# IvanTyulyandin/Spec_Viterbi

Measured on AMD Instinct MI355X. Metric: M state-updates/sec (states x obs/s) on 2405.chmm x emit_50_3500_20.ess, higher is better.
Workload: dtype f32; 1 GPU; 2405.chmm x emit_50_3500_20.ess, non-spec (min,+) step, diag kernel; states=2407, nnz=9621, sequences_per_gpu=50, observations_per_gpu=175000, state_updates_per_gpu=421225000, level=0, kernel=diag, threads=256, slots=1, fallback_rows=0, heavy_rows=2, golden_checked=False, checked_rows=0, parallelism=sequence-sharded x1 (one process per GPU, no collective)

## Files before the change

include/svh.h:

```cpp
#ifndef SPEC_VITERBI_SVH_H
#define SPEC_VITERBI_SVH_H

#include <stddef.h>
#include <stdint.h>

#ifdef __cplusplus
extern "C" {
#endif

#define SVH_ABI_VERSION 4

enum {
    SVH_OK = 0,
    SVH_E_INVALID = -1,
    SVH_E_RANGE = -2,
    SVH_E_NOMEM = -3,
    SVH_E_HIP = -4,
    SVH_E_UNSUPPORTED = -5,
    SVH_E_STATE = -6,
    SVH_E_IO = -7
};

typedef struct svh_hmm* svh_hmm_t;
typedef struct svh_ess* svh_ess_t;
typedef struct svh_model* svh_model_t;
typedef struct svh_batch* svh_batch_t;

int svh_abi_version(void);
const char* svh_last_error(void);
int svh_device_count(int* count);

int svh_hmm_read(const char* path, svh_hmm_t* out);
int svh_hmm_dims(svh_hmm_t h, uint64_t* n, uint64_t* S, uint64_t* nstart, uint64_t* ntrans);
int svh_hmm_copy(svh_hmm_t h, uint64_t* start_cols, float* start_vals, float* emissions,
                 uint64_t* trans_src, uint64_t* trans_dst, float* trans_prob);
void svh_hmm_free(svh_hmm_t h);
int svh_ess_read(const char* path, svh_ess_t* out);
int svh_ess_dims(svh_ess_t e, uint64_t* nseq, uint64_t* total_symbols);
int svh_ess_copy(svh_ess_t e, uint64_t* offsets , uint64_t* symbols);
void svh_ess_free(svh_ess_t e);

enum { SVH_KERNEL_AUTO = 0, SVH_KERNEL_FUSED = 1, SVH_KERNEL_GENERIC = 2, SVH_KERNEL_BAND = 3,
       SVH_KERNEL_CHAIN = 4, SVH_KERNEL_PIPE = 5, SVH_KERNEL_PIPE_WIDE = 6, SVH_KERNEL_SPEC2 = 7,
       SVH_KERNEL_SPEC2_PIPE = 8, SVH_KERNEL_DIAG = 9, SVH_KERNEL_SPEC2_DIAG = 10 };

typedef struct {
    int32_t device;
    int32_t kernel;
    int32_t max_threads;
    int32_t flags;
} svh_model_opts;

#define SVH_MODEL_SPEC_DENSE 1

int svh_model_create(uint64_t n, uint64_t S, uint64_t nstart, const uint64_t* start_cols,
                     const float* start_vals, const float* emissions, uint64_t ntrans,
                     const uint64_t* trans_src, const uint64_t* trans_dst,
                     const float* trans_prob, const svh_model_opts* opts, svh_model_t* out);
int svh_model_destroy(svh_model_t m);

typedef struct {
    int32_t kernel;
    int32_t family;
    int32_t threads;
    int32_t slots;
    int32_t light_terms;
    int32_t heavy_rows;
    int32_t heavy_uniform;
    int32_t device;
    uint64_t n, S, nnz;
    uint64_t lds_bytes;
    uint64_t spec_level;
    uint64_t spec_bytes;
    int32_t paths_kernel;
    int32_t wide_threads;
    int32_t wide_slots;
    uint32_t cu_count;
    int32_t pipe_slots;
    int32_t pipe_waves;
    int32_t pipe_groups;
    uint32_t pipe_max_nseq;
    int32_t pipew_slots;
    int32_t pipew_waves;
    int32_t pipew_blocks;
    uint32_t pipew_min_nseq;
    uint32_t pipe_max_nseq_paths;
    int32_t diag_ranges;
    uint32_t diag_max_nseq;
    int32_t diag_sm;
} svh_model_info;
int svh_model_get_info(svh_model_t m, svh_model_info* info);

int svh_spec_build(svh_model_t m, uint32_t level, void* stream);

enum { SVH_BATCH_PATHS = 1, SVH_BATCH_NO_TIMING = 2 };

int svh_batch_create(svh_model_t m, uint64_t nseq, const uint64_t* offsets,
                     const uint64_t* symbols, uint32_t flags, svh_batch_t* out);
int svh_batch_run(svh_batch_t b, uint32_t level, void* stream);
int svh_batch_run_time_parallel(svh_batch_t b, uint32_t seg_len, uint32_t probe_len, float rel_tol,
                                void* stream, uint64_t* fallbacks);
int svh_batch_read(svh_batch_t b, void* stream, float* scores ,
                   int64_t* best_state , int32_t* paths );
int svh_host_alloc(size_t bytes, void** out);
int svh_host_free(void* p);
int svh_batch_device_results(svh_batch_t b, float** scores, int64_t** best_state);
int svh_batch_elapsed_ms(svh_batch_t b, float* ms);
int svh_batch_step_floor_ms(svh_batch_t b, void* stream, uint32_t reps, float* ms);
int svh_batch_plan(svh_batch_t b, uint32_t level, svh_model_info* info);
int svh_batch_fallbacks(svh_batch_t b, uint64_t* rows);
int svh_batch_fallback_rows(svh_batch_t b, uint32_t* flags);
int svh_pipe_variant_built(int32_t slots, int32_t waves, int32_t table_mode, int32_t* built);
int svh_batch_destroy(svh_batch_t b);
int svh_batch_debug_fault(svh_batch_t b, void* stream);

int svh_batch_create_u8(svh_model_t m, uint64_t nseq, const uint64_t* offsets,
                        const uint8_t* symbols, uint32_t flags, svh_batch_t* out);

typedef struct svh_batchset* svh_batchset_t;
typedef struct {
    uint64_t members;
    uint64_t grouped;
    uint64_t launches;
    uint64_t grid;
    uint64_t lds_bytes;
    int32_t waves;
} svh_batchset_info;
int svh_batchset_create(const svh_model_t* models, uint64_t nmodels, uint64_t nseq,
                        const uint64_t* offsets, const uint8_t* symbols, uint32_t flags, svh_batchset_t* out);
int svh_batchset_run(svh_batchset_t s, uint32_t level, void* stream);
int svh_batchset_member(svh_batchset_t s, uint64_t i, svh_batch_t* out);
int svh_batchset_get_info(svh_batchset_t s, svh_batchset_info* info);
int svh_batchset_elapsed_ms(svh_batchset_t s, float* ms);
int svh_batchset_destroy(svh_batchset_t s);

enum { SVH_FORMAT_AUTO = 0, SVH_FORMAT_ESS = 1, SVH_FORMAT_FASTA = 2 };
typedef struct svh_reader* svh_reader_t;
int svh_reader_open(const char* path, int format, svh_reader_t* out);
int svh_reader_next(svh_reader_t r, uint64_t max_seqs, uint64_t max_symbols, uint64_t* nseq,
                    const uint64_t** offsets, const uint8_t** symbols);
void svh_reader_close(svh_reader_t r);

typedef int (*svh_result_fn)(void* user, uint64_t first_seq, uint64_t nseq, const uint64_t* offsets,
                             const float* scores, const int64_t* best_state, const int32_t* paths);
int svh_decode_file(svh_model_t m, const char* path, int format, uint32_t level, uint32_t flags,
                    uint64_t max_seqs, uint64_t max_symbols, svh_result_fn fn, void* user,
                    uint64_t* nseq_total);

int svh_viterbi(svh_model_t m, uint32_t level, uint64_t nseq, const uint64_t* offsets,
                const uint64_t* symbols, float* scores, int64_t* best_state, int32_t* paths);
int svh_viterbi_u8(svh_model_t m, uint32_t level, uint64_t nseq, const uint64_t* offsets,
                   const uint8_t* symbols, float* scores, int64_t* best_state, int32_t* paths);
int svh_viterbi_seqs(svh_model_t m, uint32_t level, uint64_t nseq, const uint64_t* const* seqs,
                     const uint64_t* lens, float* scores, int64_t* best_state, int32_t* paths);

#ifdef __cplusplus
}
#endif

#endif
```

spec_viterbi_amd/_lib.py:

```python
from __future__ import annotations

import ctypes
import os
from ctypes import POINTER, c_char_p, c_float, c_int, c_int32, c_int64, c_uint32, c_uint64, c_void_p

LIB_NAME = "libspec_viterbi_hip.so"
LIB_PATH = os.path.join(os.path.dirname(os.path.abspath(__file__)), LIB_NAME)
if os.environ.get("SVH_LIB"):
    LIB_PATH = os.path.abspath(os.environ["SVH_LIB"])

SVH_OK = 0
SVH_E_INVALID = -1
SVH_E_RANGE = -2
SVH_E_NOMEM = -3
SVH_E_HIP = -4
SVH_E_UNSUPPORTED = -5
SVH_E_STATE = -6
SVH_E_IO = -7

SVH_KERNEL_AUTO = 0
SVH_KERNEL_FUSED = 1
SVH_KERNEL_GENERIC = 2
SVH_KERNEL_BAND = 3
SVH_KERNEL_CHAIN = 4
SVH_KERNEL_PIPE = 5
SVH_KERNEL_PIPE_WIDE = 6
SVH_KERNEL_SPEC2 = 7
SVH_KERNEL_SPEC2_PIPE = 8
SVH_KERNEL_DIAG = 9
SVH_KERNEL_SPEC2_DIAG = 10
SVH_BATCH_PATHS = 1
SVH_BATCH_NO_TIMING = 2
SVH_MODEL_SPEC_DENSE = 1


class SvhError(RuntimeError):

    def __init__(self, code: int, msg: str):
        super().__init__(f"svh error {code}: {msg}")
        self.code = code


class svh_model_opts(ctypes.Structure):
    _fields_ = [("device", c_int32), ("kernel", c_int32), ("max_threads", c_int32), ("flags", c_int32)]


class svh_model_info(ctypes.Structure):
    _fields_ = [
        ("kernel", c_int32), ("family", c_int32), ("threads", c_int32), ("slots", c_int32),
        ("light_terms", c_int32), ("heavy_rows", c_int32), ("heavy_uniform", c_int32), ("device", c_int32),
        ("n", c_uint64), ("S", c_uint64), ("nnz", c_uint64), ("lds_bytes", c_uint64),
        ("spec_level", c_uint64), ("spec_bytes", c_uint64), ("paths_kernel", c_int32), ("wide_threads", c_int32),
        ("wide_slots", c_int32), ("cu_count", c_uint32), ("pipe_slots", c_int32), ("pipe_waves", c_int32),
        ("pipe_groups", c_int32), ("pipe_max_nseq", c_uint32),
        ("pipew_slots", c_int32), ("pipew_waves", c_int32), ("pipew_blocks", c_int32), ("pipew_min_nseq", c_uint32),
        ("pipe_max_nseq_paths", c_uint32),
        ("diag_ranges", c_int32),
        ("diag_max_nseq", c_uint32),
        ("diag_sm", c_int32),
    ]


class svh_batchset_info(ctypes.Structure):
    _fields_ = [("members", c_uint64), ("grouped", c_uint64), ("launches", c_uint64), ("grid", c_uint64),
                ("lds_bytes", c_uint64), ("waves", c_int32)]


P_u64 = POINTER(c_uint64)
P_f32 = POINTER(c_float)
P_i64 = POINTER(c_int64)
P_i32 = POINTER(c_int32)
P_u32 = POINTER(c_uint32)

SIGNATURES = {
    "svh_abi_version": (c_int, []),
    "svh_last_error": (c_char_p, []),
    "svh_device_count": (c_int, [P_i32]),
    "svh_hmm_read": (c_int, [c_char_p, POINTER(c_void_p)]),
    "svh_hmm_dims": (c_int, [c_void_p, P_u64, P_u64, P_u64, P_u64]),
    "svh_hmm_copy": (c_int, [c_void_p, P_u64, P_f32, P_f32, P_u64, P_u64, P_f32]),
    "svh_hmm_free": (None, [c_void_p]),
    "svh_ess_read": (c_int, [c_char_p, POINTER(c_void_p)]),
    "svh_ess_dims": (c_int, [c_void_p, P_u64, P_u64]),
    "svh_ess_copy": (c_int, [c_void_p, P_u64, P_u64]),
    "svh_ess_free": (None, [c_void_p]),
    "svh_model_create": (c_int, [c_uint64, c_uint64, c_uint64, P_u64, P_f32, P_f32, c_uint64, P_u64,
                                 P_u64, P_f32, POINTER(svh_model_opts), POINTER(c_void_p)]),
    "svh_model_destroy": (c_int, [c_void_p]),
    "svh_model_get_info": (c_int, [c_void_p, POINTER(svh_model_info)]),
    "svh_spec_build": (c_int, [c_void_p, c_uint32, c_void_p]),
    "svh_batch_create": (c_int, [c_void_p, c_uint64, P_u64, P_u64, c_uint32, POINTER(c_void_p)]),
    "svh_batch_run": (c_int, [c_void_p, c_uint32, c_void_p]),
    "svh_batch_read": (c_int, [c_void_p, c_void_p, P_f32, P_i64, P_i32]),
    "svh_host_alloc": (c_int, [ctypes.c_size_t, POINTER(c_void_p)]),
    "svh_host_free": (c_int, [c_void_p]),
    "svh_batch_device_results": (c_int, [c_void_p, POINTER(c_void_p), POINTER(c_void_p)]),
    "svh_batch_elapsed_ms": (c_int, [c_void_p, P_f32]),
    "svh_batch_step_floor_ms": (c_int, [c_void_p, c_void_p, c_uint32, P_f32]),
    "svh_batch_fallback_rows": (c_int, [c_void_p, P_u32]),
    "svh_batch_plan": (c_int, [c_void_p, c_uint32, POINTER(svh_model_info)]),
    "svh_batch_fallbacks": (c_int, [c_void_p, P_u64]),
    "svh_pipe_variant_built": (c_int, [ctypes.c_int32, ctypes.c_int32, ctypes.c_int32, POINTER(ctypes.c_int32)]),
    "svh_batch_debug_fault": (c_int, [c_void_p, c_void_p]),
    "svh_batch_destroy": (c_int, [c_void_p]),
    "svh_viterbi": (c_int, [c_void_p, c_uint32, c_uint64, P_u64, P_u64, P_f32, P_i64, P_i32]),
    "svh_viterbi_u8": (c_int, [c_void_p, c_uint32, c_uint64, P_u64, POINTER(ctypes.c_uint8), P_f32, P_i64, P_i32]),
    "svh_viterbi_seqs": (c_int, [c_void_p, c_uint32, c_uint64, P_u64, P_u64, P_f32, P_i64, P_i32]),
    "svh_batch_create_u8": (c_int, [c_void_p, c_uint64, P_u64, POINTER(ctypes.c_uint8), c_uint32, POINTER(c_void_p)]),
    "svh_batch_run_time_parallel": (c_int, [c_void_p, c_uint32, c_uint32, c_float, c_void_p, P_u64]),
    "svh_batchset_create": (c_int, [POINTER(c_void_p), c_uint64, c_uint64, P_u64, POINTER(ctypes.c_uint8), c_uint32,
                                    POINTER(c_void_p)]),
    "svh_batchset_run": (c_int, [c_void_p, c_uint32, c_void_p]),
    "svh_batchset_member": (c_int, [c_void_p, c_uint64, POINTER(c_void_p)]),
    "svh_batchset_get_info": (c_int, [c_void_p, POINTER(svh_batchset_info)]),
    "svh_batchset_elapsed_ms": (c_int, [c_void_p, P_f32]),
    "svh_batchset_destroy": (c_int, [c_void_p]),
    "svh_reader_open": (c_int, [c_char_p, c_int, POINTER(c_void_p)]),
    "svh_reader_next": (c_int, [c_void_p, c_uint64, c_uint64, P_u64, POINTER(P_u64),
                                POINTER(POINTER(ctypes.c_uint8))]),
    "svh_reader_close": (None, [c_void_p]),
    "svh_decode_file": (c_int, [c_void_p, c_char_p, c_int, c_uint32, c_uint32, c_uint64, c_uint64, c_void_p,
                                c_void_p, P_u64]),
}

SVH_FORMAT_AUTO, SVH_FORMAT_ESS, SVH_FORMAT_FASTA = 0, 1, 2
RESULT_FN = ctypes.CFUNCTYPE(c_int, c_void_p, c_uint64, c_uint64, P_u64, P_f32, P_i64, P_i32)


def _load():
    if not os.path.exists(LIB_PATH):
        raise ImportError(
            f"{LIB_PATH} not found: build the HIP extension first (python -c 'import __graft_entry__ as g; g.build()' "
            "or `make -j16`). There is no CPU fallback.")
    try:
        import torch
    except ImportError:
        pass
    lib = ctypes.CDLL(LIB_PATH)
    for name, (res, args) in SIGNATURES.items():
        fn = getattr(lib, name)
        fn.restype = res
        fn.argtypes = args
    return lib


lib = _load()


def check(rc: int) -> None:
    if rc != SVH_OK:
        msg = lib.svh_last_error()
        raise SvhError(rc, msg.decode() if msg else "")


def device_count() -> int:
    c = c_int32(0)
    check(lib.svh_device_count(ctypes.byref(c)))
    return int(c.value)


def pipe_variant_built(slots: int, waves: int, table_mode: int) -> bool:
    r = ctypes.c_int32()
    check(lib.svh_pipe_variant_built(slots, waves, table_mode, ctypes.byref(r)))
    return bool(r.value)
```

spec_viterbi_amd/csrc/diag.hip:

```cpp
#include "pipe_kernel.h"

#include <algorithm>
#include <cstdlib>

namespace svh {

namespace {

#ifndef SVH_DIAG_K
#define SVH_DIAG_K 64
#endif
constexpr uint32_t kDK = SVH_DIAG_K;
static_assert(kDK == 32 || kDK == 64, "block length");
constexpr uint32_t kDR = 5 * kDK;
constexpr uint32_t kDRS = kDR + 64;
constexpr uint32_t kDRS2 = kDR + 128;
static_assert(kDRS2 % 64 == 0, "the eb plane and the second diagonal lie whole multiples of 64 floats behind the lane's ea");
constexpr uint32_t kDG = kDR / kDK;
constexpr uint32_t kCP = kDK / 2;
constexpr uint32_t kDE = 4;
constexpr uint32_t kAG = 4;
#ifndef SVH_DIAG_PS
#define SVH_DIAG_PS 6
#endif
#ifndef SVH_DIAG_PE
#define SVH_DIAG_PE 2
#endif
constexpr uint32_t kPS = SVH_DIAG_PS;
constexpr uint32_t kPE = SVH_DIAG_PE;
constexpr uint32_t kNS = kPS + 2;
constexpr uint32_t kNE = kPE + 2;
static_assert(kPE + 2 <= kPS && kPS % 2 == 0 && kPE % 2 == 0 && kDK % kNS == 0 && kDK % kNE == 0,
              "prefetch distances: the register slots of step j (j % kNS, j % kNE) repeat every block");
static_assert(kPE == 2 && kDK % (2 * kAG) == 0,
              "address groups: read 2 kAG steps ahead into two register slots (group % 2), which repeat every block; "
              "a group's slot is free once the pairs of its last two steps are issued (kPE = 2)");
constexpr uint32_t kDMaxSym = 32;
static_assert(kDMaxSym == kDiagSetMaxSym, "kernels.h: what the runtime admits to a set launch");
#ifndef SVH_DIAG_AB
#define SVH_DIAG_AB 0
#endif
#ifndef SVH_DIAG_FINISH
#define SVH_DIAG_FINISH 0
#endif
#ifndef SVH_DIAG_PAB
#define SVH_DIAG_PAB 0
#endif
#ifndef SVH_DIAG_CMPX2
#define SVH_DIAG_CMPX2 1
#endif
#ifndef SVH_DIAG_LDPRIO
#define SVH_DIAG_LDPRIO 0
#endif
#ifndef SVH_DIAG_LDDRAIN
#define SVH_DIAG_LDDRAIN 1
#endif
#ifndef SVH_DIAG_DONE_STRIDE
#define SVH_DIAG_DONE_STRIDE 1
#endif

__device__ __forceinline__ f2 lds_ld2(uint32_t a) {
    return *(const __attribute__((address_space(3))) f2*)(size_t)a;
}
__device__ __forceinline__ float lds_ld1(uint32_t a) {
    return *(const __attribute__((address_space(3))) float*)(size_t)a;
}

__device__ __forceinline__ void check_off(float a, float b) {
    asm volatile("v_cmpx_nlt_f32_e32 vcc, %0, %1" : : "v"(a), "v"(b) : "vcc");
}
__device__ __forceinline__ void exec_collect(uint64_t& alive) {
    __builtin_amdgcn_sched_barrier(0);
    asm volatile("s_and_b64 %0, %0, exec\n\t"
                 "s_mov_b64 exec, -1\n\t"
                 "s_nop 4"
                 : "+s"(alive)
                 :
                 : "scc", "memory");
    __builtin_amdgcn_sched_barrier(0);
}

__host__ __device__ constexpr size_t diag_lds_main(uint32_t W, uint32_t S, bool sx, uint32_t dm = 1, bool ld = false) {
    return ((size_t)S * (dm == 2 ? kDRS2 : kDRS) * 2 + (size_t)S * 8 + (size_t)W * (ld ? 3 : 2) * kDK * (kDE + 1 + (sx ? 1 : 0)) + 2 * W) * 4;
}

constexpr uint32_t kFS = 8;
static_assert(kDK % kFS == 0 && 32 % kFS == 0 && kFS * 8 == 64, "fold: lane l reduces 8 lanes of step l / 8");
__host__ __device__ constexpr size_t diag_lds_paths(uint32_t W, uint32_t S, bool sx) {
    return ((diag_lds_main(W, S, sx) + 15) & ~(size_t)15) + (size_t)W * kFS * 64 * 4;
}

template <int W, bool SX, bool PATHS = false, int DM = 1, bool LD = false, bool FL = false>
__global__ __launch_bounds__(64 * (W + (LD ? 1 : 0))) __attribute__((amdgpu_waves_per_eu(2)))
void diag_viterbi_kernel(PipeModel m, FusedBatch b, PipeScratch x) {
    const uint32_t bx = blockIdx.x;
#include "diag_body.h"
}

template <class T>
__device__ __forceinline__ void in_global1(T*& p) {
    auto g = (__attribute__((address_space(1))) T*)p;
    asm volatile("" : "+s"(g));
    p = (T*)g;
}
template <class... T>
__device__ __forceinline__ void in_global(T*&... p) {
    (in_global1(p), ...);
}
template <int W>
__global__ __launch_bounds__(64 * W) __attribute__((amdgpu_waves_per_eu(2)))
void diag_set_kernel(const DiagSetEntry* __restrict__ e, const uint32_t* __restrict__ first, uint32_t ne) {
    constexpr bool SX = false, PATHS = false, LD = false, FL = false;
    constexpr int DM = 1;
    const uint32_t lane = threadIdx.x & 63u, gbx = blockIdx.x;
    uint32_t cnt = 0;
    for (uint32_t i0 = 0; i0 < ne; i0 += 64) {
        const uint32_t i = i0 + lane;
        const bool le = i < ne && first[i] <= gbx;
        const uint32_t c = (uint32_t)__builtin_popcountll(__builtin_amdgcn_ballot_w64(le));
        cnt += c;
        if (c < 64) break;
    }
    if (cnt == 0) return;
    const uint32_t i = (uint32_t)uniform((int)(cnt - 1));
    const uint32_t f0 = first[i];
    DiagSetEntry ent = e[i];
    in_global(ent.m.tab, ent.m.e0, ent.m.start, ent.m.lrow, ent.m.hc, ent.m.dtab, ent.m.pflags, ent.m.spos, ent.m.stamps, ent.m.dtab2);
    in_global(ent.b.symbols, ent.b.sym_off, ent.b.begin, ent.b.end, ent.b.v_in, ent.b.v_in_row, ent.b.scores, ent.b.best,
              ent.b.run_mask, ent.b.fault);
    in_global(ent.x.ctr, ent.x.done, ent.x.part, ent.x.gran, ent.x.cons, ent.x.viol, ent.x.xcc);
    const PipeModel& m = ent.m;
    const FusedBatch& b = ent.b;
    const PipeScratch& x = ent.x;
    const uint32_t bx = gbx - f0;
    {
#include "diag_body.h"
    }
}

template <bool SX>
__global__ __launch_bounds__(256) void diag_finish_kernel(PipeModel m, FusedBatch b, PipeScratch x) {
    extern __shared__ __attribute__((aligned(16))) float lds[];
    const uint32_t q = blockIdx.x, tid = threadIdx.x, lane = tid & 63u;
    uint32_t* flag = reinterpret_cast<uint32_t*>(lds + 2 * (size_t)m.P + 8);
    if (tid < 64) {
        float C = kInf, bv = kInf;
        uint32_t bk = kNoRow, vi = 0;
        for (uint32_t u = lane; u < m.nrng; u += 64) {
            const uint64_t* pu = x.part + ((size_t)q * x.G + u) * 2;
            const uint64_t a = pu[0], k2 = pu[1];
            C = fminf(C, __builtin_bit_cast(float, (uint32_t)a));
            vi |= (uint32_t)(a >> 32);
            if (k2 != ~0ull) lex_min(bv, bk, lex_key_value(k2), lex_key_index(k2));
        }
        C = wave_min63(C);
        wave_lexmin63(bv, bk);
        const bool any = __builtin_amdgcn_ballot_w64(vi != 0) != 0;
        if (lane == 63) {
            float* out = b.scores + (size_t)q * m.n;
            if (m.rowF >= 0) lex_min(bv, bk, out[m.rowF], (uint32_t)m.rowF);
            if (m.rowS >= 0) {
                out[m.rowS] = C;
                lex_min(bv, bk, C, (uint32_t)m.rowS);
            }
            if (b.best) b.best[q] = bk == kNoRow ? -1 : (int64_t)bk;
            x.viol[q] = any ? 1u : 0u;
            *flag = any ? 1u : 0u;
        }
    }
    __syncthreads();
    if (*flag) pipe_rerun_row<2, 4, SX>(m, b, q, lds);
}

template <int W, int DM = 1>
const void* diag_ptr(bool sx) {
    return sx ? reinterpret_cast<const void*>(&diag_viterbi_kernel<W, true, false, DM>)
              : reinterpret_cast<const void*>(&diag_viterbi_kernel<W, false, false, DM>);
}
template <int W, int DM>
const void* diag_loader_ptr(bool sx) {
    if constexpr (SVH_DIAG_AB != 0 || SVH_DIAG_FINISH != 0) {
        return nullptr;
    } else {
        return sx ? reinterpret_cast<const void*>(&diag_viterbi_kernel<W, true, false, DM, true>)
                  : reinterpret_cast<const void*>(&diag_viterbi_kernel<W, false, false, DM, true>);
    }
}
template <int DM>
const void* diag_floor_ptr(bool sx) {
    if constexpr (SVH_DIAG_AB != 0 || SVH_DIAG_FINISH != 0) {
        return nullptr;
    } else {
        return sx ? reinterpret_cast<const void*>(&diag_viterbi_kernel<4, true, false, DM, true, true>)
                  : reinterpret_cast<const void*>(&diag_viterbi_kernel<4, false, false, DM, true, true>);
    }
}
template <int W>
const void* diag_paths_ptr() {
    static_assert(kDK == 64, "the path records' block layout (two mask words, two checkpoints per block)");
    return reinterpret_cast<const void*>(&diag_viterbi_kernel<W, false, true>);
}

}

uint32_t diag_waves_for(uint64_t nseq) { return nseq >= 4 ? 4u : nseq >= 2 ? 2u : 1u; }

static size_t diag_lds(uint32_t W, uint32_t S, uint32_t P, bool sx, uint32_t dm = 1, bool ld = false) {
    const size_t rerun = (2 * (size_t)P + 2 * W) * 4;
    const size_t mainb = diag_lds_main(W, S, sx, dm, ld);
    return mainb > rerun ? mainb : rerun;
}

size_t diag_lds_bytes(uint32_t W, uint32_t S, uint32_t P, uint32_t dm, bool ld) { return diag_lds(W, S, P, true, dm, ld); }

uint32_t diag_sm_for(const PipeModel& m, uint64_t nseq, bool resumed, bool paths) {
    if (paths || !m.dtab2 || !m.nrng2 || SVH_DIAG_AB != 0 || SVH_DIAG_FINISH != 0) return 1;
    if (m.dsm == 1 || m.dsm == 2) return m.dsm;
    if (resumed || !m.cus) return 1;
    const uint64_t W = diag_waves_for(nseq);
    return (nseq + W - 1) / W * W * m.nrng > 4ull * m.cus ? 2 : 1;
}

bool diag_loader_for(const PipeModel& m, uint64_t nseq, bool resumed, bool paths) {
    if (paths || !nseq || SVH_DIAG_AB != 0 || SVH_DIAG_FINISH != 0 || m.dld == 1) return false;
    const uint32_t W = diag_waves_for(nseq);
    const uint32_t dm = diag_sm_for(m, nseq, resumed, paths);
    if (diag_lds(W, m.S, m.P, m.sx != 0, dm, true) > 160 * 1024) return false;
    if (m.dld == 3) return W == 4;
    if (m.dld == 2) return true;
    return m.cus && (nseq + W - 1) / W * (dm == 2 ? m.nrng2 : m.nrng) <= m.cus;
}

size_t diag_paths_lds_bytes(uint32_t W, uint32_t S, bool sx) { return diag_lds_paths(W, S, sx); }

bool diag_paths_fit(uint32_t S, bool sx) {
    return !sx && SVH_DIAG_AB == 0 && SVH_DIAG_FINISH == 0 && kDK == 64 && S > 0 && S <= kDMaxSym &&
           diag_lds_paths(4, S, sx) <= kDiagPathsLdsMax;
}

hipError_t launch_diag(const PipeModel& m, const FusedBatch& b, const PipeScratch& x, hipStream_t stream) {
    const bool paths = b.cmask != nullptr;
    if (!m.dtab || m.nrng == 0 || m.SM != 2 || m.S == 0 || m.S > kDMaxSym || (size_t)m.nrng * 64 > m.P || m.wide ||
        b.run_mask || (b.v_in && !b.v_in_row) || !x.part || !x.done || !x.viol || b.nseq > x.rows || x.G < m.nrng)
        return hipErrorInvalidValue;
    if (paths && (!b.cmask_off || !b.ckpt || !b.ckpt_off || !b.fck || !b.fck_off || !b.hrec || !b.hrec_off || !b.prec ||
                  !b.prec_off || b.v_in || !m.ties_heavy || !diag_paths_fit(m.S, m.sx != 0)))
        return hipErrorInvalidValue;
    if (b.nseq == 0) return hipSuccess;
    const uint32_t W = diag_waves_for(b.nseq);
    const uint32_t dm = diag_sm_for(m, b.nseq, b.v_in != nullptr, paths);
    if (dm == 2 && ((size_t)m.nrng2 * 128 != m.P || x.G < m.nrng2)) return hipErrorInvalidValue;
    const bool sx = m.sx != 0;
    const bool ld = diag_loader_for(m, b.nseq, b.v_in != nullptr, paths);
    const void* fn = paths     ? (W == 4 ? diag_paths_ptr<4>() : W == 2 ? diag_paths_ptr<2>() : diag_paths_ptr<1>())
                     : ld && m.dld == 3 ? (dm == 2 ? diag_floor_ptr<2>(sx) : diag_floor_ptr<1>(sx))
                     : ld      ? (dm == 2 ? (W == 4 ? diag_loader_ptr<4, 2>(sx) : W == 2 ? diag_loader_ptr<2, 2>(sx) : diag_loader_ptr<1, 2>(sx))
                                          : (W == 4 ? diag_loader_ptr<4, 1>(sx) : W == 2 ? diag_loader_ptr<2, 1>(sx) : diag_loader_ptr<1, 1>(sx)))
                     : dm == 2 ? (W == 4 ? diag_ptr<4, 2>(sx) : W == 2 ? diag_ptr<2, 2>(sx) : diag_ptr<1, 2>(sx))
                               : (W == 4 ? diag_ptr<4>(sx) : W == 2 ? diag_ptr<2>(sx) : diag_ptr<1>(sx));
    size_t lds = paths ? diag_lds_paths(W, m.S, sx) : diag_lds(W, m.S, m.P, sx, dm, ld);
    if (lds > 160 * 1024) return hipErrorInvalidValue;
    const uint64_t grid = ((uint64_t)b.nseq + W - 1) / W * (dm == 2 ? m.nrng2 : m.nrng);
    if (grid > 0x7FFFFFFFull) return hipErrorInvalidValue;
    if (m.cus) {
        const uint64_t per_cu = (grid + m.cus - 1) / m.cus;
        if (per_cu * lds <= 160 * 1024) {
            const size_t cap = (160 * 1024 / per_cu) & ~(size_t)511;
            lds = cap > lds ? cap : lds;
        }
    }
    if (lds > 64 * 1024) {
        const hipError_t e = hipFuncSetAttribute(fn, hipFuncAttributeMaxDynamicSharedMemorySize, (int)lds);
        if (e != hipSuccess) return e;
    }
    PipeModel mm = m;
    FusedBatch bb = b;
    PipeScratch xx = x;
    void* args[] = {&mm, &bb, &xx};
    const hipError_t e = hipLaunchKernel(fn, dim3((uint32_t)grid), dim3(64 * (W + (ld ? 1 : 0))), args, lds, stream);
#if SVH_DIAG_FINISH
    if (e != hipSuccess) return e;
    const void* fin = m.sx ? reinterpret_cast<const void*>(&diag_finish_kernel<true>)
                           : reinterpret_cast<const void*>(&diag_finish_kernel<false>);
    return hipLaunchKernel(fin, dim3(b.nseq), dim3(256), args, (2 * (size_t)m.P + 8 + 1) * 4, stream);
#else
    return e;
#endif
}

hipError_t diag_set_plan(const DiagSetEntry* host, const uint32_t* first_host, uint32_t ne, DiagSetLaunch* out) {
    if (!host || !first_host || !out || ne == 0 || first_host[0] != 0 || SVH_DIAG_AB != 0 || SVH_DIAG_FINISH != 0)
        return hipErrorInvalidValue;
    const uint32_t nseq = host[0].b.nseq;
    if (nseq == 0) return hipErrorInvalidValue;
    const uint32_t W = diag_waves_for(nseq);
    size_t lds = 0;
    for (uint32_t i = 0; i < ne; ++i) {
        const PipeModel& m = host[i].m;
        const FusedBatch& b = host[i].b;
        const PipeScratch& x = host[i].x;
        if (!m.dtab || m.nrng == 0 || m.SM != 2 || m.S == 0 || m.S > kDMaxSym || (size_t)m.nrng * 64 > m.P || m.wide ||
            m.sx || b.run_mask || b.cmask || (b.v_in && !b.v_in_row) || !x.part || !x.done || !x.viol || b.nseq != nseq ||
            b.nseq > x.rows || x.G < m.nrng || !b.symbols || !b.sym_off || !b.begin || !b.end || !b.scores)
            return hipErrorInvalidValue;
        const uint64_t blocks = ((uint64_t)nseq + W - 1) / W * m.nrng;
        if (first_host[i + 1] < first_host[i] || (uint64_t)first_host[i + 1] - first_host[i] != blocks) return hipErrorInvalidValue;
        lds = std::max(lds, diag_lds(W, m.S, m.P, false));
    }
    if (first_host[ne] > 0x7FFFFFFFu || lds > 160 * 1024) return hipErrorInvalidValue;
    out->grid = first_host[ne];
    out->lds_bytes = lds;
    out->waves = W;
    return hipSuccess;
}

hipError_t launch_diag_set(const DiagSetEntry* host, const uint32_t* first_host, uint32_t ne, const DiagSetEntry* entries,
                           const uint32_t* first, uint32_t cus, hipStream_t stream) {
    DiagSetLaunch L{};
    const hipError_t pe = diag_set_plan(host, first_host, ne, &L);
    if (pe != hipSuccess) return pe;
    if (!entries || !first) return hipErrorInvalidValue;
    const void* fn = L.waves == 4   ? reinterpret_cast<const void*>(&diag_set_kernel<4>)
                     : L.waves == 2 ? reinterpret_cast<const void*>(&diag_set_kernel<2>)
                                    : reinterpret_cast<const void*>(&diag_set_kernel<1>);
    size_t lds = L.lds_bytes;
    if (cus) {
        const uint64_t per_cu = (L.grid + cus - 1) / cus;
        if (per_cu * lds <= 160 * 1024) {
            const size_t cap = (160 * 1024 / per_cu) & ~(size_t)511;
            lds = cap > lds ? cap : lds;
        }
    }
    if (lds > 64 * 1024) {
        const hipError_t e = hipFuncSetAttribute(fn, hipFuncAttributeMaxDynamicSharedMemorySize, (int)lds);
        if (e != hipSuccess) return e;
    }
    const DiagSetEntry* ea = entries;
    const uint32_t* fa = first;
    uint32_t na = ne;
    void* args[] = {&ea, &fa, &na};
    return hipLaunchKernel(fn, dim3((uint32_t)L.grid), dim3(64 * L.waves), args, lds, stream);
}

}
```

spec_viterbi_amd/csrc/diag_body.h:

```cpp
    static_assert(DM == 1 || (DM == 2 && !PATHS), "decoded paths keep one diagonal per lane");
    static_assert(!LD || (!PATHS && SVH_DIAG_AB == 0 && SVH_DIAG_FINISH == 0), "the loader wave: scores only");
    static_assert(!FL || LD, "the floor is a loader-wave launch");
    constexpr uint32_t NB = LD ? 3 : 2;
    extern __shared__ __attribute__((aligned(16))) float lds[];
    constexpr uint32_t RW = 64 * DM;
    constexpr uint32_t RS = DM == 2 ? kDRS2 : kDRS;
    const uint32_t S = m.S, NR = DM == 2 ? m.nrng2 : m.nrng, NP = NR * RW, P = m.P;
    float* ring = lds;
    float* hcr = ring + (size_t)S * RS * 2;
    float* strm = hcr + S * 8;
    float* adr = strm + W * NB * kDK * kDE;
    float* xsf = adr + W * NB * kDK;
    uint32_t* wnb = reinterpret_cast<uint32_t*>(xsf + (SX ? W * NB * kDK : 0));
    uint32_t* rrow = wnb + W;

    const uint32_t tid = threadIdx.x, lane = tid & 63u;
    const uint32_t w = (uint32_t)uniform((int)(tid >> 6));
    const uint32_t rg = bx % NR, grp = bx / NR;
    const uint32_t q = grp * W + w;
    const bool ldr = LD && w == W;
    constexpr bool flr = FL;
    const bool real = (!LD || w < W) && q < b.nseq;
    const uint32_t ring_a = lds_addr(ring);

    for (uint32_t i = tid; i < S * 8; i += 64 * (W + (LD ? 1 : 0))) {
        const uint32_t o = i >> 3, k = i & 7u;
        const float* h = m.hc + o * 8;
        float v = 0.0f;
        if (k == 0) v = h[1];
        else if (k == 1) v = h[0];
        else if (k == 2) v = h[3];
        else if (k == 3) v = h[2];
        else if (k == 4) v = SX ? h[4] : kInf;
        else if (k == 5) v = __builtin_bit_cast(float, ring_a + o * RS * 8u);
        hcr[i] = v;
    }

    const uint8_t* __restrict__ sym = b.symbols + (real ? b.sym_off[q] : 0);
    const uint32_t len = real ? (uint32_t)uniform((int)b.end[q]) : 0u;
    const uint32_t beg = real ? (uint32_t)uniform((int)b.begin[q]) : 0u;
    const uint32_t first = beg ? beg : 1u;
    const uint32_t nst = len > first ? len - first : 0u;
    const uint32_t nb = (nst + kDK - 1) / kDK;
    if (lane == 0 && (!LD || w < W)) {
        wnb[w] = nb;
        rrow[w] = kNoRow;
    }

    constexpr uint32_t kT = 64 * W;
    constexpr uint32_t kRep = (kCP * kDMaxSym + kT - 1) / kT;
    const uint32_t nchunk = kCP * S;
    typedef float lvec __attribute__((ext_vector_type(4 * kRep)));
    lvec lreg;
    auto gload = [&](uint32_t g) {
        const uint32_t c0 = (rg * RW + g * kDK) % NP;
#pragma unroll
        for (uint32_t r = 0; r < kRep; ++r) {
            const uint32_t k = min(tid + r * kT, nchunk - 1);
            const float4 v = DM == 2 ? *reinterpret_cast<const float4*>(m.dtab2 + (size_t)(k / (kCP / 2)) * NP + c0 + 4 * (k % (kCP / 2)))
                                     : *reinterpret_cast<const float4*>(m.dtab + (size_t)(k / kCP) * NP + c0 + 2 * (k % kCP));
            lreg[4 * r] = v.x;
            lreg[4 * r + 1] = v.y;
            lreg[4 * r + 2] = v.z;
            lreg[4 * r + 3] = v.w;
        }
    };
    auto lwrite = [&](uint32_t g) {
        const uint32_t s0 = (g % kDG) * kDK;
#pragma unroll
        for (uint32_t r = 0; r < kRep; ++r) {
            const uint32_t k = tid + r * kT;
            if (k < nchunk) {
                float* d = DM == 2 ? ring + (size_t)(k / (kCP / 2)) * kDRS2 + s0 + 4 * (k % (kCP / 2))
                                   : ring + ((size_t)(k / kCP) * kDRS + s0 + 2 * (k % kCP)) * 2;
                const float4 v = make_float4(lreg[4 * r], lreg[4 * r + 1], lreg[4 * r + 2], lreg[4 * r + 3]);
                *reinterpret_cast<float4*>(d) = v;
                if (s0 < RW) *reinterpret_cast<float4*>(d + kDR * (DM == 2 ? 1 : 2)) = v;
            }
        }
    };
    uint32_t symv = 0;
    auto symload = [&](uint32_t kb) {
        const uint32_t t = first + kb * kDK + lane;
        const uint32_t tc = t < len ? t : (len ? len - 1 : 0u);
        symv = (real && lane < kDK) ? (uint32_t)sym[tc] : 0u;
    };
    auto sbuild = [&](uint32_t kb) {
        if (lane < kDK) {
            const uint32_t o = symv < S ? symv : 0u;
            const float4 h0 = *reinterpret_cast<const float4*>(hcr + o * 8);
            const float2 h1 = *reinterpret_cast<const float2*>(hcr + o * 8 + 4);
            const uint32_t i = kb * kDK + 1 + lane;
            const uint32_t e = (w * 2 + (kb & 1u)) * kDK + lane;
            *reinterpret_cast<float4*>(strm + e * kDE) = h0;
            adr[e] = __builtin_bit_cast(float, __builtin_bit_cast(uint32_t, h1.y) + (i % kDR) * (DM == 2 ? 4u : 8u));
            if (SX) xsf[e] = h1.x;
        }
    };
    constexpr uint32_t kRepL = kCP * kDMaxSym / 64;
    typedef float lvecl __attribute__((ext_vector_type(LD ? 4 * kRepL : 4)));
    lvecl lregl = 0.0f;
    const uint8_t* lsym[W] = {};
    uint32_t llen[W] = {}, lfirst[W] = {}, lsymv[W] = {};
    bool lreal[W] = {};
    auto gloadl = [&](uint32_t g) {
        if constexpr (LD) {
            const uint32_t c0 = (rg * RW + g * kDK) % NP;
#pragma unroll
            for (uint32_t r = 0; r < kRepL; ++r) {
                if (r * 64 < nchunk) {
                    const uint32_t k = min(lane + r * 64, nchunk - 1);
                    const float4 v = DM == 2 ? *reinterpret_cast<const float4*>(m.dtab2 + (size_t)(k / (kCP / 2)) * NP + c0 + 4 * (k % (kCP / 2)))
                                             : *reinterpret_cast<const float4*>(m.dtab + (size_t)(k / kCP) * NP + c0 + 2 * (k % kCP));
                    lregl[4 * r] = v.x;
                    lregl[4 * r + 1] = v.y;
                    lregl[4 * r + 2] = v.z;
                    lregl[4 * r + 3] = v.w;
                }
            }
        }
    };
    auto lwritel = [&](uint32_t g) {
        if constexpr (LD) {
            const uint32_t s0 = (g % kDG) * kDK;
#pragma unroll
            for (uint32_t r = 0; r < kRepL; ++r) {
                const uint32_t k = lane + r * 64;
                if (k < nchunk) {
                    float* d = DM == 2 ? ring + (size_t)(k / (kCP / 2)) * kDRS2 + s0 + 4 * (k % (kCP / 2))
                                       : ring + ((size_t)(k / kCP) * kDRS + s0 + 2 * (k % kCP)) * 2;
                    const float4 v = make_float4(lregl[4 * r], lregl[4 * r + 1], lregl[4 * r + 2], lregl[4 * r + 3]);
                    *reinterpret_cast<float4*>(d) = v;
                    if (s0 < RW) *reinterpret_cast<float4*>(d + kDR * (DM == 2 ? 1 : 2)) = v;
                }
            }
        }
    };
    auto symloadl = [&](uint32_t kb) {
#pragma unroll
        for (int u = 0; u < W; ++u) {
            const uint32_t t = lfirst[u] + kb * kDK + lane;
            const uint32_t tc = t < llen[u] ? t : (llen[u] ? llen[u] - 1 : 0u);
            lsymv[u] = (lreal[u] && lane < kDK) ? (uint32_t)lsym[u][tc] : 0u;
        }
    };
    auto sbuildl = [&](uint32_t kb) {
        if (lane < kDK) {
            const uint32_t i = kb * kDK + 1 + lane;
            const uint32_t ro = (i % kDR) * (DM == 2 ? 4u : 8u);
            const uint32_t e0 = (kb % NB) * kDK + lane;
#pragma unroll
            for (int u = 0; u < W; ++u) {
                const uint32_t o = lsymv[u] < S ? lsymv[u] : 0u;
                const float4 h0 = *reinterpret_cast<const float4*>(hcr + o * 8);
                const float2 h1 = *reinterpret_cast<const float2*>(hcr + o * 8 + 4);
                const uint32_t e = u * NB * kDK + e0;
                *reinterpret_cast<float4*>(strm + e * kDE) = h0;
                adr[e] = __builtin_bit_cast(float, __builtin_bit_cast(uint32_t, h1.y) + ro);
                if (SX) xsf[e] = h1.x;
            }
        }
    };
    if constexpr (LD) {
        if (ldr) {
#pragma unroll
            for (int u = 0; u < W; ++u) {
                const uint32_t qu = grp * W + u;
                lreal[u] = qu < b.nseq;
                lsym[u] = b.symbols + (lreal[u] ? b.sym_off[qu] : 0);
                llen[u] = lreal[u] ? (uint32_t)uniform((int)b.end[qu]) : 0u;
                const uint32_t bu = lreal[u] ? (uint32_t)uniform((int)b.begin[qu]) : 0u;
                lfirst[u] = bu ? bu : 1u;
            }
        }
    }

#if SVH_DIAG_AB == 6
    return;
#endif
    if constexpr (LD) {
        if (ldr) {
            gloadl(4);
            symloadl(0);
        } else {
            gload(0);
            lwrite(0);
            gload(1);
            lwrite(1);
            gload(2);
            lwrite(2);
            gload(3);
            lwrite(3);
        }
        __syncthreads();
        if (ldr) {
            sbuildl(0);
            symloadl(1);
            sbuildl(1);
            symloadl(2);
            if (flr) {
                sbuildl(2);
                lwritel(4);
            }
        }
    } else {
#if SVH_DIAG_AB != 4
    gload(0);
    lwrite(0);
    gload(1);
    lwrite(1);
    gload(2);
    lwrite(2);
    gload(3);
    lwrite(3);
    gload(4);
#endif
    symload(0);
    __syncthreads();
    sbuild(0);
    symload(1);
    }

    const uint32_t Lg = rg * 64 + lane;
    const uint32_t nck = len ? (len - 1) / kDiagCkptEvery + 1 : 0u;
    uint32_t* dmq = nullptr;
    float *ckq = nullptr, *fckq = nullptr, *cckq = nullptr, *pmq = nullptr, *fr_wr = nullptr;
    const float* fr_rd = nullptr;
    uint32_t pcur = Lg;
    if constexpr (PATHS) {
        float* fring = lds + ((diag_lds_main(W, S, SX) + 15) & ~(size_t)15) / 4 + w * kFS * 64;
        fr_wr = fring + lane;
        fr_rd = fring + lane * 8;
        if (real) {
            dmq = b.cmask + b.cmask_off[q] + Lg;
            ckq = b.ckpt + b.ckpt_off[q];
            fckq = b.fck + b.fck_off[q];
            cckq = reinterpret_cast<float*>(b.hrec + b.hrec_off[q]) + (size_t)rg * nck;
            pmq = reinterpret_cast<float*>(b.prec) + b.prec_off[q] + (size_t)rg * len + (lane >> 3);
        }
    }

    float xv = kInf, xv2 = kInf, F = kInf, c = kInf;
    uint64_t alive = ~0ull;
    if (real && beg == 0) {
        const uint32_t o0 = (uint32_t)uniform((int)sym[0]);
        const uint32_t p = rg * RW + lane;
        xv = m.e0[(size_t)o0 * P + p] + m.start[p];
        if (DM == 2) xv2 = m.e0[(size_t)o0 * P + p + 64] + m.start[p + 64];
        F = m.rowF >= 0 ? m.hc[o0 * 8 + 5] + m.startF : kInf;
        c = (rg == 0 && lane == 0 && m.rowS >= 0) ? m.hc[o0 * 8 + 6] + m.startS : kInf;
    } else if (real) {
        const float* vin = b.v_in + (size_t)b.v_in_row[q] * m.n;
        const uint32_t r = m.lrow[rg * RW + lane];
        xv = r != kNoRow ? vin[r] : kInf;
        if (DM == 2) {
            const uint32_t r2 = m.lrow[rg * RW + 64 + lane];
            xv2 = r2 != kNoRow ? vin[r2] : kInf;
        }
        F = m.rowF >= 0 ? vin[m.rowF] : kInf;
        c = (rg == 0 && lane == 0 && m.rowS >= 0) ? vin[m.rowS] : kInf;
    }
    if constexpr (PATHS) {
        if (real) {
            ckq[Lg] = xv;
            float mu0 = xv, c0 = c;
            wave_min63x2(mu0, c0);
            if (lane == 63) {
                pmq[-7] = mu0;
                cckq[0] = c0;
            }
            if (rg == 0 && lane == 0) fckq[0] = F;
        }
    }
    __syncthreads();
    uint32_t nbmax = 0;
#pragma unroll
    for (int u = 0; u < W; ++u) nbmax = wnb[u] > nbmax ? wnb[u] : nbmax;
    nbmax = (uint32_t)uniform((int)nbmax);

    typedef float hvec __attribute__((ext_vector_type(4 * kNS)));
    typedef float avec __attribute__((ext_vector_type(2 * kAG)));
    typedef float evec __attribute__((ext_vector_type(2 * DM * kNE)));
    hvec hq;
    avec aq, xq;
    evec eq;
    auto spos = [&](uint32_t kb, uint32_t j) {
        if constexpr (LD) return (w * NB + (j < kDK ? kb : kb + 1) % NB) * kDK + j % kDK;
        const uint32_t e0 = (w * 2 + (kb & 1u)) * kDK;
        return (j < kDK ? e0 : e0 ^ kDK) + j % kDK;
    };
    auto sread = [&](uint32_t kb, uint32_t j, uint32_t slot) {
        const float4 h = *reinterpret_cast<const float4*>(strm + spos(kb, j) * kDE);
        hq[4 * slot] = h.x;
        hq[4 * slot + 1] = h.y;
        hq[4 * slot + 2] = h.z;
        hq[4 * slot + 3] = h.w;
    };
    auto gread = [&](avec& q, const float* src, uint32_t kb, uint32_t j) {
        const float4 g = *reinterpret_cast<const float4*>(src + spos(kb, j));
        const uint32_t slot = (j / kAG) % 2;
        q[4 * slot] = g.x;
        q[4 * slot + 1] = g.y;
        q[4 * slot + 2] = g.z;
        q[4 * slot + 3] = g.w;
    };
    auto eread = [&](uint32_t j) {
        const float roff = aq[j % (2 * kAG)];
        if constexpr (DM == 2) {
            const uint32_t a = __builtin_bit_cast(uint32_t, roff) + lane * 4u;
            eq[4 * (j % kNE)] = lds_ld1(a);
            eq[4 * (j % kNE) + 1] = lds_ld1(a + 256u);
            eq[4 * (j % kNE) + 2] = lds_ld1(a + kDRS2 * 4u);
            eq[4 * (j % kNE) + 3] = lds_ld1(a + kDRS2 * 4u + 256u);
            return;
        }
        const f2 e = lds_ld2(__builtin_bit_cast(uint32_t, roff) + lane * 8u);
        eq[2 * (j % kNE)] = e.x;
        eq[2 * (j % kNE) + 1] = e.y;
    };
#pragma unroll
    for (uint32_t j = 0; j < kPS; ++j) sread(0, j, j);
    gread(aq, adr, 0, 0);
    gread(aq, adr, 0, kAG);
    if (SX) gread(xq, xsf, 0, 0);
#pragma unroll
    for (uint32_t j = 0; j < kPE; ++j) eread(j);

    f2 FC = (f2){F, c};
    f2 XP = (f2){xv, 0.0f};
    uint32_t dw = 0;
    auto step = [&](const float4& h, float xs, const f2& e, uint32_t slot = 0) {
        const f2 Y = XP.xx + (f2){h.x, h.y};
        const f2 Wv = FC + (f2){h.z, h.w};
        const float za = e.x + FC.x;
        const float zb = e.y + XP.x;
        float cn = fminf(Wv.y, Y.y);
        if (SX) cn = fminf(cn, xs + FC.x);
        check_off(Y.x, Wv.x);
        if constexpr (PATHS && SVH_DIAG_PAB != 1) push_le(dw, za, zb);
        XP.x = fminf(zb, za);
        FC = (f2){Wv.x, cn};
        if constexpr (PATHS && SVH_DIAG_PAB != 2) fr_wr[slot * 64] = XP.x;
    };
    f2 X2 = (f2){xv, xv2};
    uint32_t nviol = 0;
    auto step2 = [&](const float4& h, float xs, const f2& ea, const f2& eb) {
        XP.x = fminf(X2.x, X2.y);
        const f2 Y = XP.xx + (f2){h.x, h.y};
        const f2 Wv = FC + (f2){h.z, h.w};
        const f2 za = ea + FC.xx;
        const f2 zb = eb + X2;
        float cn = fminf(Wv.y, Y.y);
        if (SX) cn = fminf(cn, xs + FC.x);
        if (SVH_DIAG_CMPX2) check_off(Y.x, Wv.x);
        else nviol += Y.x < Wv.x ? 1u : 0u;
        X2 = (f2){fminf(zb.x, za.x), fminf(zb.y, za.y)};
        FC = (f2){Wv.x, cn};
    };
    float4 fa0 = make_float4(kInf, kInf, kInf, kInf), fa1 = fa0;
    auto fold_read = [&]() {
        if (SVH_DIAG_PAB == 2) return;
        __builtin_amdgcn_fence(__ATOMIC_SEQ_CST, "wavefront");
        fa0 = *reinterpret_cast<const float4*>(fr_rd);
        fa1 = *reinterpret_cast<const float4*>(fr_rd + 4);
        __builtin_amdgcn_fence(__ATOMIC_SEQ_CST, "wavefront");
    };
    auto fold_min = [&](uint32_t t0, uint32_t n) {
        if (SVH_DIAG_PAB == 2) return;
        uint32_t tv = t0;
        float4 a0 = fa0, a1 = fa1;
        asm volatile("" : "+v"(tv), "+v"(a0.x), "+v"(a0.y), "+v"(a0.z), "+v"(a0.w), "+v"(a1.x), "+v"(a1.y), "+v"(a1.z), "+v"(a1.w));
        float mn = fminf(fminf(fminf(a0.x, a0.y), fminf(a0.z, a0.w)), fminf(fminf(a1.x, a1.y), fminf(a1.z, a1.w)));
        const uint32_t inf = 0x7f800000u;
        mn = fminf(mn, __builtin_bit_cast(float, dpp_u<0xB1>(__builtin_bit_cast(uint32_t, mn), inf)));
        mn = fminf(mn, __builtin_bit_cast(float, dpp_u<0x4E>(__builtin_bit_cast(uint32_t, mn), inf)));
        mn = fminf(mn, __builtin_bit_cast(float, dpp_u<0x141>(__builtin_bit_cast(uint32_t, mn), inf)));
        if ((lane & 7u) == 0 && (lane >> 3) < n) pmq[tv] = mn;
    };
    auto fold = [&](uint32_t t0, uint32_t n) {
        fold_read();
        fold_min(t0, n);
    };
    uint32_t dw0 = 0;
    float xs0 = kInf, fs0 = kInf, cs0 = kInf;
    auto keep32 = [&]() {
        dw0 = dw;
        xs0 = XP.x;
        fs0 = FC.x;
        cs0 = FC.y;
    };
    auto block_records = [&](uint32_t kb, uint32_t rem) {
        if (SVH_DIAG_PAB == 3) {
            asm volatile("" : : "v"(dw0), "v"(dw), "v"(xs0), "v"(fs0), "v"(cs0));
            return;
        }
        uint32_t kv = kb, pc = pcur;
        float cn1 = cs0, cn2 = FC.y;
        asm volatile("" : "+v"(kv), "+v"(pc), "+v"(cn1), "+v"(cn2));
        const uint32_t w0 = rem > 32 ? dw0 : dw << (32u - rem);
        dmq[(size_t)(2 * kv) * NP] = w0;
        if (rem > 32) dmq[(size_t)(2 * kv + 1) * NP] = dw << (64u - rem);
        if (rem >= 32) {
            const bool two = rem == 64;
            uint32_t p1 = pc + 32;
            p1 = p1 >= NP ? p1 - NP : p1;
            uint32_t p2 = p1 + 32;
            p2 = p2 >= NP ? p2 - NP : p2;
            const float x1 = rem > 32 ? xs0 : XP.x, f1 = rem > 32 ? fs0 : FC.x;
            float c1 = rem > 32 ? cn1 : cn2, c2 = cn2;
            ckq[(size_t)(2 * kv + 1) * NP + p1] = x1;
            if (two) ckq[(size_t)(2 * kv + 2) * NP + p2] = XP.x;
            wave_min63x2(c1, c2);
            if (lane == 63) {
                cckq[2 * kv + 1] = c1;
                if (two) cckq[2 * kv + 2] = c2;
            }
            if (rg == 0 && lane == 0) {
                fckq[2 * kv + 1] = f1;
                if (two) fckq[2 * kv + 2] = FC.x;
            }
            pcur = p2;
        }
    };
    auto blockwork = [&](uint32_t kb) {
        lwrite(kb + 4);
        gload(kb + 5);
        sbuild(kb + 1);
        symload(kb + 2);
    };
    auto block = [&](uint32_t kb) {
        __builtin_amdgcn_sched_barrier(0);
#pragma unroll
        for (uint32_t j = 0; j < kDK; ++j) {
            const uint32_t a = (SVH_DIAG_AB == 1 || FL) ? 0u : j % kNS, b2 = FL ? 0u : j % kNE;
            const float4 h = make_float4(hq[4 * a], hq[4 * a + 1], hq[4 * a + 2], hq[4 * a + 3]);
            const float xs = SX ? xq[(SVH_DIAG_AB == 1 || FL) ? 0u : j % (2 * kAG)] : 0.0f;
            const f2 e = DM == 2 ? (f2){eq[4 * b2], eq[4 * b2 + 1]} : (f2){eq[2 * b2], eq[2 * b2 + 1]};
            if (j % 2 == 0) {
                if (SVH_DIAG_AB != 1 && !FL) {
                    sread(kb, j + kPS, (j + kPS) % kNS);
                    sread(kb, j + kPS + 1, (j + kPS + 1) % kNS);
                }
                if (SVH_DIAG_AB != 2 && !FL) {
                    eread(j + kPE);
                    eread(j + kPE + 1);
                }
                if (SVH_DIAG_AB != 1 && !FL && j % kAG == 0) {
                    gread(aq, adr, kb, j + 2 * kAG);
                    if (SX) gread(xq, xsf, kb, j + kAG);
                }
                if (SVH_DIAG_AB == 0 && !FL) {
                    __builtin_amdgcn_s_waitcnt(0xC07F | (((SX ? 6 : 5) + (PATHS ? 2 : 0) + (DM == 2 ? 2 : 0)) << 8));
                    __builtin_amdgcn_sched_barrier(0);
                }
            }
            if constexpr (DM == 2) step2(h, xs, e, (f2){eq[4 * b2 + 2], eq[4 * b2 + 3]});
            else step(h, xs, e, j % kFS);
            if (j % 2 == 1) __builtin_amdgcn_sched_barrier(0);
            if constexpr (PATHS) {
                if (j % kFS == kFS - 1 && (SVH_DIAG_PAB != 4 || j == kDK - 1)) {
                    exec_collect(alive);
                    if (SVH_DIAG_PAB == 4) {
                        fold(kb * kDK + 1 + j - (kFS - 1), kFS);
                    } else {
                        if (j >= kFS) fold_min(kb * kDK + 1 + j - (2 * kFS - 1), kFS);
                        fold_read();
                        if (j == kDK - 1) fold_min(kb * kDK + 1 + j - (kFS - 1), kFS);
                    }
                    if (j == 31) keep32();
                    if (j == kDK - 1) block_records(kb, kDK);
                    __builtin_amdgcn_sched_barrier(0);
                }
            }
        }
        if constexpr (!PATHS) exec_collect(alive);
    };
    auto tail = [&](uint32_t kb, uint32_t rem) {
        const uint32_t e0 = LD ? (w * NB + kb % NB) * kDK : (w * 2 + (kb & 1u)) * kDK;
        if constexpr (PATHS) {
            for (uint32_t g0 = 0; g0 < rem; g0 += kFS) {
                const uint32_t n = rem - g0 < kFS ? rem - g0 : kFS;
                __builtin_amdgcn_sched_barrier(0);
                for (uint32_t j = g0; j < g0 + n; ++j) {
                    const float4 h = *reinterpret_cast<const float4*>(strm + (e0 + j) * kDE);
                    const float roff = adr[e0 + j];
                    step(h, SX ? xsf[e0 + j] : 0.0f, lds_ld2(__builtin_bit_cast(uint32_t, roff) + lane * 8u), j - g0);
                }
                exec_collect(alive);
                fold(kb * kDK + 1 + g0, n);
                if (g0 + n == 32 && rem > 32) keep32();
            }
            block_records(kb, rem);
            return;
        }
        __builtin_amdgcn_sched_barrier(0);
        for (uint32_t j = 0; j < rem; ++j) {
            const float4 h = *reinterpret_cast<const float4*>(strm + (e0 + j) * kDE);
            const float roff = adr[e0 + j];
            if constexpr (DM == 2) {
                const uint32_t a = __builtin_bit_cast(uint32_t, roff) + lane * 4u;
                step2(h, SX ? xsf[e0 + j] : 0.0f, (f2){lds_ld1(a), lds_ld1(a + 256u)},
                      (f2){lds_ld1(a + kDRS2 * 4u), lds_ld1(a + kDRS2 * 4u + 256u)});
            } else {
                step(h, SX ? xsf[e0 + j] : 0.0f, lds_ld2(__builtin_bit_cast(uint32_t, roff) + lane * 8u));
            }
        }
        exec_collect(alive);
    };

    if constexpr (LD) {
        if (ldr) {
            for (uint32_t k = 0; k < nbmax; ++k) {
                if (!flr) {
                    sbuildl(k + 2);
                    symloadl(k + 3);
                    lwritel(k + 4);
                    gloadl(k + 5);
                }
                lds_barrier();
            }
            return;
        }
        if (SVH_DIAG_LDPRIO) __builtin_amdgcn_s_setprio(SVH_DIAG_LDPRIO);
    }
    for (uint32_t k = 0; k < nbmax; ++k) {
        const uint32_t rem = k < nb ? nst - k * kDK : 0u;
        const bool full = k < nb && rem >= kDK;
        if constexpr (!LD) blockwork(k);
        if (k < nb) {
#ifdef SVH_DIAG_SIMPLE
            tail(k, rem >= kDK ? kDK : rem);
#else
            if (full) block(k);
            else tail(k, rem);
#endif
        }
        if (LD && !SVH_DIAG_LDDRAIN) asm volatile("s_barrier" ::: "memory");
        else if (SVH_DIAG_AB != 3) lds_barrier();
    }

    if (DM == 2 && !SVH_DIAG_CMPX2) alive &= __builtin_amdgcn_ballot_w64(nviol == 0);
    F = FC.x;
    c = FC.y;
    xv = DM == 2 ? X2.x : XP.x;
    xv2 = X2.y;

#if SVH_DIAG_AB == 5
    if (real && m.lrow[(rg * 64 + lane + nst) % NP] != kNoRow)
        g_st_score(b.scores + (size_t)q * m.n + m.lrow[(rg * 64 + lane + nst) % NP], xv);
    return;
#endif
#if SVH_DIAG_FINISH
    if (real) {
        float* out = b.scores + (size_t)q * m.n;
        const uint32_t r = m.lrow[(rg * 64 + lane + nst) % NP];
        float bv = kInf;
        uint32_t bk = kNoRow;
        if (r != kNoRow) {
            out[r] = xv;
            bv = xv;
            bk = r;
        }
        wave_lexmin63(bv, bk);
        const float cmin = wave_min63(c);
        const bool any_viol = alive != ~0ull;
        if (lane == 63) {
            uint64_t* part = x.part + ((size_t)q * x.G + rg) * 2;
            part[0] = ((uint64_t)(any_viol ? 1u : 0u) << 32) | __builtin_bit_cast(uint32_t, cmin);
            part[1] = lex_key(bv, bk);
            if (rg == 0 && m.rowF >= 0) out[m.rowF] = F;
        }
    }
    return;
#endif
    uint32_t last = 0;
    if (real) {
        float* out = b.scores + (size_t)q * m.n;
        const uint32_t pe = (rg * RW + lane + nst) % NP;
        const uint32_t r = m.lrow[pe];
        float bv = kInf;
        uint32_t bk = kNoRow;
        if (r != kNoRow) {
            g_st_score(out + r, xv);
            bv = xv;
            bk = r;
        }
        if constexpr (DM == 2) {
            const uint32_t r2 = m.lrow[pe + 64 >= NP ? pe + 64 - NP : pe + 64];
            if (r2 != kNoRow) {
                g_st_score(out + r2, xv2);
                lex_min(bv, bk, xv2, r2);
            }
        }
        wave_lexmin63(bv, bk);
        const float cmin = wave_min63(c);
        const bool any_viol = alive != ~0ull;
        if (lane == 63 && !flr) {
            uint64_t* part = x.part + ((size_t)q * x.G + rg) * 2;
            g_st64(part, ((uint64_t)(any_viol ? 1u : 0u) << 32) | __builtin_bit_cast(uint32_t, cmin));
            g_st64(part + 1, lex_key(bv, bk));
#if SVH_DIAG_AB == 7
            last = rg == NR - 1 ? 1u : 0u;
#else
            asm volatile("s_waitcnt vmcnt(0)" ::: "memory");
            const uint32_t d = __hip_atomic_fetch_add(x.done + (size_t)q * SVH_DIAG_DONE_STRIDE, 1u, __ATOMIC_RELAXED, __HIP_MEMORY_SCOPE_AGENT);
            last = d == NR - 1 ? 1u : 0u;
#endif
#if SVH_DIAG_AB == 8
            last = 0;
#endif
        }
        last = readlane_u(last, 63);
    }
    if (last) {
        float C = kInf, bv2 = kInf;
        uint32_t bk2 = kNoRow, vi = 0;
        for (uint32_t u = lane; u < NR; u += 64) {
            const uint64_t* pu = x.part + ((size_t)q * x.G + u) * 2;
            const uint64_t a = g_ld64(pu), k2 = g_ld64(pu + 1);
            C = fminf(C, __builtin_bit_cast(float, (uint32_t)a));
            vi |= (uint32_t)(a >> 32);
            if (k2 != ~0ull) lex_min(bv2, bk2, lex_key_value(k2), lex_key_index(k2));
        }
        C = wave_min63(C);
        wave_lexmin63(bv2, bk2);
        const bool any = __builtin_amdgcn_ballot_w64(vi != 0) != 0;
        if (lane == 63) {
            float* out = b.scores + (size_t)q * m.n;
            if (m.rowF >= 0) {
                out[m.rowF] = F;
                lex_min(bv2, bk2, F, (uint32_t)m.rowF);
            }
            if (m.rowS >= 0) {
                out[m.rowS] = C;
                lex_min(bv2, bk2, C, (uint32_t)m.rowS);
            }
            if (b.best) b.best[q] = bk2 == kNoRow ? -1 : (int64_t)bk2;
            x.viol[q] = any ? 1u : 0u;
            __hip_atomic_store(x.done + (size_t)q * SVH_DIAG_DONE_STRIDE, 0u, __ATOMIC_RELAXED, __HIP_MEMORY_SCOPE_AGENT);
            if (any && !PATHS) rrow[w] = q;
        }
    }
    if constexpr (PATHS) return;
    __syncthreads();
    uint32_t rq[W];
#pragma unroll
    for (int u = 0; u < W; ++u) rq[u] = rrow[u];
#pragma unroll
    for (int u = 0; u < W; ++u) {
        if (rq[u] != kNoRow) {
            __syncthreads();
            pipe_rerun_row<2, W, SX>(m, b, rq[u], lds);
        }
    }
```

spec_viterbi_amd/csrc/kernels.h:

```cpp
#pragma once

#include <hip/hip_runtime.h>

#include <cstddef>
#include <cstdint>

namespace svh {

constexpr int kMaxHeavy = 4;
constexpr int kMaxExc = 4;
constexpr int kMaxWaves = 16;
constexpr uint32_t kNoPred = 0xFFFFu;
constexpr uint32_t kSymChunk = 4096;
constexpr uint32_t kSymPad = 64;
constexpr int kMaxFusedThreads = 512;

enum HeavyMode : int { kHeavyGeneral = 0, kHeavyUniform = 1 };

struct FusedModel {
    const float* emis;
    const float* start;
    const uint32_t* lcol;
    const float* lval;
    const float* hval;
    const uint8_t* hvalid;
    const float* hmask;
    int hrow[kMaxHeavy];
    float hw[kMaxHeavy];
    uint32_t xk[kMaxHeavy][kMaxExc];
    float xw[kMaxHeavy][kMaxExc];
    uint32_t H;
    uint32_t n;
    uint32_t S;
    uint32_t slots;
    uint32_t estride;
    uint32_t vstride;
    uint32_t B;
};

constexpr uint32_t kFaultPipe = 1u, kFaultPipeWide = 2u, kFaultChain = 4u;

struct FusedBatch {
    const uint8_t* symbols;
    const uint64_t* sym_off;
    const uint32_t* begin;
    const uint32_t* end;
    const float* v_in;
    const uint32_t* v_in_row;
    float* scores;
    int64_t* best;
    uint16_t* bp;
    const uint64_t* bp_off;
    uint32_t* cmask;
    const uint64_t* cmask_off;
    uint32_t* hrec;
    const uint64_t* hrec_off;
    float* ckpt;
    const uint64_t* ckpt_off;
    float2* prec;
    const uint64_t* prec_off;
    float* fck;
    const uint64_t* fck_off;
    const uint32_t* run_mask;
    const struct PipeScratch* pipe;
    uint32_t* fault;
    uint32_t nseq;
};

constexpr int kBandHeavy = 2;
constexpr int kMaxBandThreads = 1024;
constexpr int kDefaultBandThreads = 512;
constexpr int kBandTailA = 0;
constexpr int kBandTailX = kBandHeavy;
constexpr int kBandTailE = kBandHeavy + kBandHeavy * kBandHeavy;
constexpr int kBandTail = 8;
constexpr int band_tail_x(int h, int k) { return kBandTailX + (h == k ? h : kBandHeavy + h); }
static_assert(kBandHeavy == 2, "band_tail_x assumes two heavy rows");
static_assert(kBandTailE + kBandHeavy <= kBandTail, "band row tail");

struct BandModel {
    const float* erows;
    const float* erows_t;
    const float* start;
    const float* aw;
    const float* bw;
    const uint32_t* lrow;
    int hrow[kBandHeavy];
    int hvalid[kBandHeavy];
    float hstart[kBandHeavy];
    uint32_t n, S, B, SM, erow, H;
    uint32_t ge;
    uint32_t dbg;
    unsigned long long* stamps;
    const uint8_t* pflags;
    const int32_t* spos;
    uint32_t hx_exist;
    uint32_t hl_exist;
    uint32_t ties_heavy;
};
constexpr int kBandStamps = 8;

constexpr int kChainMaxSym = 32;
constexpr int kChainMaxThreads = 512;
constexpr uint32_t kChainSymChunk = 32768;
constexpr int kChainRing = 8;
inline size_t chain_lds_bytes() {
    return (size_t)kChainMaxSym * kBandTail * sizeof(float) + (size_t)kChainRing * 2 * kMaxWaves * 8 +
           3 * kChainRing * 4 + 2 * kMaxWaves * sizeof(float) + kChainSymChunk;
}
bool chain_supported(int sm, int waves, int ha, bool ge);
bool chain_paths_supported(int sm, int waves);
hipError_t launch_chain(const BandModel& m, int ha, const FusedBatch& b, hipStream_t stream);
hipError_t launch_chain_traceback(const BandModel& m, const FusedBatch& b, const uint64_t* path_off,
                                  int32_t* paths, hipStream_t stream);
inline uint64_t chain_mask_words(uint64_t len, uint32_t waves, uint32_t sm) {
    return len > 1 ? (len - 1 + 31) / 32 * (uint64_t)sm * 64 * waves : 0;
}
constexpr uint32_t kPathRing = 64;
constexpr uint32_t kRecWords = 4;
inline size_t chain_path_lds_bytes() { return (size_t)kPathRing * kRecWords * 4; }
inline uint64_t chain_hrec_words(uint64_t len) { return len > 1 ? (len - 1) * kRecWords : 0; }
constexpr uint32_t kCkptEvery = 16;
inline uint64_t chain_ckpt_floats(uint64_t len, uint32_t sm, uint32_t threads) {
    return len ? ((len - 1) / kCkptEvery + 1) * (uint64_t)sm * threads : 0;
}

constexpr int kPipeRing = 32;
constexpr int kPipeGroup = 8;
constexpr int kPipeGRing = 256;
constexpr int kPipeAhead = 4;
constexpr int kPipeWindow = 1024;
struct PipeModel {
    const float2* tab;
    const float* e0;
    const float* start;
    const uint32_t* lrow;
    const float* hc;
    int rowF, rowS;
    float startF, startS;
    uint32_t n, S, P, nblk, SM, W, G;
    uint32_t cus;
    uint32_t sx;
    uint32_t tm;
    uint32_t wide;
    float emax2;
    const float2* dtab;
    uint32_t nrng;
    uint32_t rerun;
    const uint8_t* pflags;
    const int32_t* spos;
    uint32_t hx_exist;
    uint32_t hl_exist;
    uint32_t ties_heavy;
    unsigned long long* stamps;
    uint32_t diag;
    uint32_t dld;
    const float* dtab2;
    uint32_t nrng2;
    uint32_t dsm;
};
constexpr int kPipeStamps = 15;
constexpr uint32_t kCtrClass = 4, kCtrLeft = 12, kCtrWords = 16;
struct PipeScratch {
    uint32_t* ctr;
    uint32_t* done;
    uint64_t* part;
    uint64_t* gran;
    uint32_t* cons;
    uint32_t* viol;
    uint32_t* xcc;
    uint32_t xmap;
    uint32_t rows, G;
};
constexpr uint32_t kPairSymbols = 20;
__host__ __device__ inline size_t pipe_lds_bytes(uint32_t W, uint32_t S) {
    return ((size_t)W * kPipeRing * 64 + 16 + (size_t)S * 8 + (size_t)W * 4 + 4) * 4;
}
__host__ __device__ inline bool pipe_rerun_fits(uint32_t P, uint32_t W) {
    return 2ull * P + 2ull * W <= (size_t)W * kPipeRing * 64;
}
bool pipe_supported(int sm, int waves, bool sx);
bool pipe_tm_supported(int tm);
hipError_t launch_pipe(const PipeModel& m, const FusedBatch& b, const PipeScratch& x, hipStream_t stream,
                       bool step_floor = false);
hipError_t launch_pipe_l2(const PipeModel& m, const FusedBatch& b, const PipeScratch& x, hipStream_t stream);
bool pipe_l2_supported(const PipeModel& m);
bool pipe_paths_supported(int sm, int waves);
hipError_t launch_pipe_traceback(const PipeModel& m, const FusedBatch& b, const uint64_t* path_off, int32_t* paths,
                                 const uint32_t* skip, hipStream_t stream);
constexpr uint32_t kPipeTbMaxP = 2560;
inline uint64_t pipe_mask_words(uint64_t len, uint32_t nblk, uint32_t sm) {
    return len > 1 ? (len - 1 + 31) / 32 * (uint64_t)nblk * sm * 64 : 0;
}
__host__ __device__ inline uint32_t pipe_prec_parts(bool wide) { (void)wide; return 1u; }
inline uint64_t pipe_prec_count(uint64_t len, uint32_t nblk, uint32_t parts) { return (uint64_t)nblk * parts * len; }
inline uint64_t pipe_ckpt_floats(uint64_t len, uint32_t P) { return len ? ((len - 1) / kCkptEvery + 1) * (uint64_t)P : 0; }
inline uint64_t pipe_fck_floats(uint64_t len) { return len ? (len - 1) / 32 + 1 : 0; }
constexpr uint32_t kPRingStride = 132;
constexpr uint32_t kPPlane = 260;
constexpr uint32_t kPQuadStride = 520;
inline size_t pipe_path_lds_bytes(uint32_t W) { return (size_t)W * 8 * kPQuadStride * 4; }
uint32_t diag_waves_for(uint64_t nseq);
size_t diag_lds_bytes(uint32_t W, uint32_t S, uint32_t P, uint32_t dm = 1, bool ld = false);
uint32_t diag_sm_for(const PipeModel& m, uint64_t nseq, bool resumed, bool paths);
bool diag_loader_for(const PipeModel& m, uint64_t nseq, bool resumed, bool paths);
hipError_t launch_diag(const PipeModel& m, const FusedBatch& b, const PipeScratch& x, hipStream_t stream);
constexpr uint32_t kDiagSetMaxSym = 32;
struct DiagSetEntry {
    PipeModel m;
    FusedBatch b;
    PipeScratch x;
};
struct DiagSetLaunch {
    uint64_t grid;
    size_t lds_bytes;
    uint32_t waves;
};
hipError_t diag_set_plan(const DiagSetEntry* host, const uint32_t* first_host, uint32_t ne, DiagSetLaunch* out);
hipError_t launch_diag_set(const DiagSetEntry* host, const uint32_t* first_host, uint32_t ne, const DiagSetEntry* entries,
                           const uint32_t* first, uint32_t cus, hipStream_t stream);
bool diag_l2_supported(const PipeModel& m);
size_t diag_l2_lds_bytes(uint32_t W, uint32_t S);
hipError_t launch_diag_l2(const PipeModel& m, const FusedBatch& b, const PipeScratch& x, hipStream_t stream);
constexpr uint32_t kDiagCkptEvery = 32;
constexpr size_t kDiagPathsLdsMax = 80 * 1024;
inline uint64_t diag_mask_words(uint64_t len, uint32_t nrng) { return len > 1 ? (len - 1 + 31) / 32 * (uint64_t)nrng * 64 : 0; }
inline uint64_t diag_ckpt_floats(uint64_t len, uint32_t nrng) {
    return len ? ((len - 1) / kDiagCkptEvery + 1) * (uint64_t)nrng * 64 : 0;
}
inline uint64_t diag_mu_floats(uint64_t len, uint32_t nrng) { return (uint64_t)nrng * len; }
inline uint64_t diag_cck_floats(uint64_t len, uint32_t nrng) { return len ? ((len - 1) / 32 + 1) * (uint64_t)nrng : 0; }
size_t diag_paths_lds_bytes(uint32_t W, uint32_t S, bool sx);
bool diag_paths_fit(uint32_t S, bool sx);
hipError_t launch_diag_traceback(const PipeModel& m, const FusedBatch& b, const uint64_t* path_off, int32_t* paths,
                                 const uint32_t* skip, hipStream_t stream);

__host__ __device__ inline uint32_t pipew_chunks(uint32_t SM, bool sx) { return SM / 2 + 1 + (sx ? 1 : 0); }
inline size_t pipew_lds_bytes(uint32_t SM, uint32_t W, uint32_t S, bool sx, bool paths = false) {
    return (size_t)S * pipew_chunks(SM, sx) * 64 * 16 + (size_t)W * 8 * 64 * 4 + 16 +
           (paths ? (size_t)W * 8 * kPRingStride * 4 : 0);
}
bool pipew_supported(int sm, int waves, bool sx);
uint32_t pipew_paths_waves_max(uint32_t sm, uint32_t S, bool sx);
bool pipew_paths_supported(int sm, uint32_t S, bool sx);
inline uint32_t pipew_waves_for(const PipeModel& m, uint64_t nseq) {
    const uint64_t need = (nseq * m.nblk + m.cus - 1) / (m.cus ? m.cus : 1);
    static const uint32_t ws[] = {1, 2, 4, 8, 12, 16};
    uint32_t w = m.W;
    for (uint32_t c : ws)
        if (c >= need) {
            w = c < m.W ? c : m.W;
            break;
        }
    return w;
}
hipError_t launch_pipew(const PipeModel& m, const FusedBatch& b, const PipeScratch& x, hipStream_t stream);

struct CsrModel {
    const float* emis;
    const float* start;
    const uint32_t* rowptr;
    const uint32_t* col;
    const float* val;
    const uint32_t* row_of;
    uint32_t n;
    uint32_t S;
    uint32_t nnz;
};

enum FusedFamily : int {
    kFamR2Uni = 0,
    kFamR2 = 1,
    kFamR4 = 2,
    kFamR8 = 3,
    kFamR16 = 4,
    kNumFamilies = 5
};
int family_rmax(int fam);
int family_hmax(int fam);
int family_xmax(int fam);
int family_mode(int fam);
constexpr int kSlotChoices[] = {1, 2, 3, 4, 5, 6, 8, 10, 12, 16};
constexpr int kNumSlotChoices = 10;

const void* fused_kernel_r2uni(int smax, bool paths);
const void* fused_kernel_r2(int smax, bool paths);
const void* fused_kernel_r4(int smax, bool paths);
const void* fused_kernel_r8(int smax, bool paths);
const void* fused_kernel_r16(int smax, bool paths);

inline size_t fused_lds_bytes_for(int sm, uint32_t B, uint32_t vstride) {
    const size_t ndma = (size_t)(sm + 3) / 4;
    return (3 * (size_t)vstride + 3 * ndma * B * 4) * sizeof(float) +
           3 * kMaxHeavy * sizeof(uint64_t) + 2 * kMaxWaves * sizeof(float) + kSymChunk + 64 + 16;
}
inline size_t fused_lds_bytes(const FusedModel& m) {
    return fused_lds_bytes_for((int)m.slots, m.B, m.vstride);
}
constexpr size_t kMaxLdsBytes = 160 * 1024;

hipError_t launch_fused(const FusedModel& m, const FusedBatch& b, int fam, bool paths,
                        hipStream_t stream);
constexpr int kBandSlotChoices[] = {1, 2, 3, 4, 5, 6, 8, 10, 12, 16};
constexpr int kNumBandSlotChoices = 10;
inline size_t band_lds_bytes(uint32_t erow) {
    return (3 * (size_t)erow + 4 * kMaxWaves + 2 * kMaxWaves) * sizeof(float) + kSymChunk + 64 + 16;
}
hipError_t launch_band(const BandModel& m, int ha, const FusedBatch& b, hipStream_t stream);
size_t generic_lds_bytes(uint32_t n);
hipError_t launch_generic(const CsrModel& m, const FusedBatch& b, int threads, bool paths,
                          hipStream_t stream);
hipError_t launch_traceback(const FusedBatch& b, const uint64_t* path_off, int32_t* paths,
                            uint32_t n, hipStream_t stream);

hipError_t launch_spec_fold(const CsrModel& m, float* mfold, hipStream_t stream);
hipError_t launch_spec_densify(const CsrModel& m, const float* mfold, float* h1, uint32_t pstride,
                               hipStream_t stream);
hipError_t launch_spec_extend(const CsrModel& m, const float* mfold, const float* h_prev,
                              uint64_t kprev, float* h_new, uint32_t pstride, hipStream_t stream);
struct SpecChunkBatch {
    const uint8_t* symbols;
    const uint64_t* sym_off;
    const uint32_t* nchunks;
    const float* v_src;
    float* v_dst;
    uint32_t nseq;
    uint32_t level;
    uint32_t chunk;
};
hipError_t launch_spec_chunk(const CsrModel& m, const float* products, const SpecChunkBatch& c,
                             uint32_t pstride, hipStream_t stream);
constexpr uint32_t kSpec2Threads = 1024;
constexpr uint32_t kSpec2LightMax = 4;
struct Spec2Model {
    const float* emis;
    const uint32_t* la;
    const uint32_t* lb;
    const float* lv;
    const uint32_t* thr;
    const uint32_t* tcp;
    const uint32_t* ha;
    const uint32_t* hb;
    const float* hv;
    const uint32_t* hrow;
    const float* amax;
    uint32_t n, S, H, NP;
    uint32_t R, KL, NHS;
    uint32_t nhs;
    uint32_t prune;
    unsigned long long* stamps;
};
constexpr int kSpec2Stamps = 8;
struct Spec2Batch {
    const uint8_t* symbols;
    const uint64_t* sym_off;
    const uint32_t* len;
    const uint32_t* nchunks;
    float* v;
// ... 61 lines not shown
```

spec_viterbi_amd/csrc/runtime.cpp:

```cpp
#include "runtime.h"

#include <algorithm>
#include <chrono>
#include <cmath>
#include <cstdio>
#include <cstdlib>
#include <cstring>
#include <functional>
#include <limits>
#include <map>
#include <memory>
#include <numeric>

namespace svh {

namespace {

constexpr float kInfH = std::numeric_limits<float>::infinity();

uint32_t round_up(uint32_t x, uint32_t m) { return (x + m - 1) / m * m; }

uint32_t float_bits(float f) {
    uint32_t u;
    std::memcpy(&u, &f, 4);
// ... 494 lines not shown
    if (ge) {
        const uint32_t smp = (SM + 3) / 4 * 4;
        bp.erows_t.assign((size_t)S * B * smp, kInfH);
        for (uint32_t o = 0; o < S; ++o)
            for (uint32_t p = 0; p < nL; ++p)
                bp.erows_t[((size_t)o * B + p / SM) * smp + p % SM] = hm.emis[(size_t)o * n + light[p]];
    }
    bp.erows.assign((size_t)S * erow, kInfH);
    for (uint32_t o = 0; o < S; ++o) {
        const float* E = hm.emis.data() + (size_t)o * n;
        float* row = bp.erows.data() + (size_t)o * erow;
        for (uint32_t p = 0; p < nL; ++p) row[slot_of(p)] = E[light[p]];
        float* tl = row + cap;
        for (int x = 0; x < kBandHeavy; ++x) {
            if (!bp.hvalid[x]) continue;
            const float eh = E[bp.hrow[x]];
            tl[kBandTailA + x] = eh + wh[x];
            for (const auto& [src, w] : exc[x]) tl[band_tail_x((int)x, (int)src)] = eh + w;
            tl[kBandTailE + x] = eh;
        }
    }
    return bp;
}

void DeviceBandPlan::upload(const BandPlan& p, uint32_t n, uint32_t S, hipStream_t s) {
    plan = p;
    if (!p.ok) return;
    d_erows.upload(p.erows.data(), p.erows.size() * 4, s);
    d_start.upload(p.start.data(), p.start.size() * 4, s);
    d_aw.upload(p.aw.data(), p.aw.size() * 4, s);
    d_bw.upload(p.bw.data(), p.bw.size() * 4, s);
    d_lrow.upload(p.lrow.data(), p.lrow.size() * 4, s);
    if (p.ge) d_erows_t.upload(p.erows_t.data(), p.erows_t.size() * 4, s);
    d_pflags.upload(p.pflags.data(), p.pflags.size(), s);
    d_spos.upload(p.spos.data(), p.spos.size() * 4, s);
    std::memset(&view, 0, sizeof(view));
    view.erows = d_erows.as<float>();
    view.start = d_start.as<float>();
    view.aw = d_aw.as<float>();
    view.bw = d_bw.as<float>();
    view.lrow = d_lrow.as<uint32_t>();
    view.erows_t = p.ge ? d_erows_t.as<float>() : nullptr;
    view.ge = p.ge ? 1u : 0u;
    view.pflags = d_pflags.as<uint8_t>();
    view.spos = d_spos.as<int32_t>();
    view.hx_exist = p.hx_exist;
    view.hl_exist = p.hl_exist;
    view.ties_heavy = p.ties_heavy ? 1u : 0u;
    for (int h = 0; h < kBandHeavy; ++h) {
        view.hrow[h] = p.hrow[h];
        view.hvalid[h] = p.hvalid[h];
        view.hstart[h] = p.hstart[h];
    }
    view.n = n;
    view.S = S;
    view.B = p.B;
    view.SM = p.SM;
    view.erow = p.erow;
    view.H = p.H;
    const char* dbg = std::getenv("SVH_BAND_DEBUG");
    view.dbg = dbg ? (uint32_t)std::atoi(dbg) : 0u;
    if (view.dbg & (4u | 128u)) {
        d_stamps.alloc((size_t)4096 * kMaxWaves * kBandStamps * 8);
        hip_check(hipMemsetAsync(d_stamps.ptr, 0, d_stamps.bytes, s), "stamps");
        view.stamps = d_stamps.as<unsigned long long>();
    }
}

PipePlan make_pipe_plan(const HostModel& hm, uint32_t sm, uint32_t waves, bool wide) {
    PipePlan pp;
    const uint32_t n = hm.n, S = hm.S;
    if (S > 32) return pp;
    const BandShape sh = analyze_band(hm);
    if (!sh.ok || sh.HA != 1) return pp;
    const uint32_t H = (uint32_t)sh.heavy.size();
    float xff = kInfH, xss = kInfH, xsf = kInfH;
    for (const auto& e : sh.exc[0]) {
        if (e.first != 0) return pp;
        xff = e.second;
    }
    bool sx = false;
    if (H == 2) {
        for (const auto& e : sh.exc[1]) {
            if (e.first == 1) xss = e.second;
            else { xsf = e.second; sx = true; }
        }
    }
    if (const char* e = std::getenv(wide ? "SVH_PIPEW_SM" : "SVH_PIPE_SM")) sm = (uint32_t)std::atoi(e);
    if (const char* e = std::getenv(wide ? "SVH_PIPEW_WAVES" : "SVH_PIPE_WAVES")) waves = (uint32_t)std::atoi(e);
    if (sm == 0) sm = wide ? 8 : 2;
    if (waves == 0) waves = wide ? 16 : 4;
    if (wide ? !pipew_supported((int)sm, (int)waves, sx) : !pipe_supported((int)sm, (int)waves, sx)) return pp;
    if (wide && pipew_lds_bytes(sm, waves, S, sx) > 160 * 1024) return pp;
    const uint32_t nL = (uint32_t)sh.light.size();
    const uint32_t bsz = 64 * sm;
    pp.wide = wide;
    pp.SM = sm;
    pp.W = waves;
    pp.nblk = (nL + bsz - 1) / bsz;
    pp.G = wide ? pp.nblk : (pp.nblk + waves - 1) / waves;
    pp.P = pp.nblk * bsz;
    pp.sx = sx;
    pp.rowF = (int)sh.heavy[0];
    pp.rowS = H == 2 ? (int)sh.heavy[1] : -1;
    pp.startF = hm.start[sh.heavy[0]];
    pp.startS = H == 2 ? hm.start[sh.heavy[1]] : kInfH;
    const uint32_t P = pp.P;
    const uint32_t nc = wide ? pipew_chunks(sm, sx) : 0;
    pp.tab.assign(wide ? (size_t)pp.nblk * S * nc * 64 * 4 : (size_t)pp.nblk * S * sm * 64 * 2, kInfH);
    pp.e0.assign((size_t)S * P, kInfH);
    pp.start.assign(P, kInfH);
    pp.lrow.assign(P, 0xFFFFFFFFu);
    for (uint32_t p = 0; p < nL; ++p) {
        const uint32_t j = sh.light[p], blk = p / bsz, lane = (p % bsz) / sm, s = p % sm;
        pp.start[p] = hm.start[j];
        pp.lrow[p] = j;
        for (uint32_t o = 0; o < S; ++o) {
            const float e = hm.emis[(size_t)o * n + j];
            pp.e0[(size_t)o * P + p] = e;
            const float eb = e + sh.bw[p];
            const float ea = e + sh.aw[0][p];
            if (wide) {
                const uint32_t ib = s == 0 ? sm - 1 : s - 1, ia = sm + s;
                float* base = pp.tab.data() + (((size_t)blk * S + o) * nc) * 64 * 4;
                base[((ib / 4) * 64 + lane) * 4 + ib % 4] = eb;
                base[((ia / 4) * 64 + lane) * 4 + ia % 4] = ea;
            } else {
                float* t = pp.tab.data() + ((((size_t)blk * S + o) * sm + s) * 64 + lane) * 2;
                t[0] = eb;
                t[1] = ea;
            }
        }
    }
    if (!wide && sm == 2) {
        pp.nrng = (nL + 63) / 64;
        const uint32_t NP = pp.nrng * 64;
        pp.dtab.assign((size_t)S * NP * 2, kInfH);
        for (uint32_t p = 0; p < nL; ++p)
            for (uint32_t o = 0; o < S; ++o) {
                const float e = hm.emis[(size_t)o * n + sh.light[p]];
                float* d = pp.dtab.data() + ((size_t)o * NP + p) * 2;
                d[0] = e + sh.aw[0][p];
                d[1] = e + sh.bw[p];
            }
        pp.nrng2 = (nL + 127) / 128;
        const uint32_t NP2 = pp.nrng2 * 128;
        pp.dtab2.assign((size_t)S * 2 * NP2, kInfH);
        for (uint32_t p = 0; p < nL; ++p)
            for (uint32_t o = 0; o < S; ++o) {
                const float* d = pp.dtab.data() + ((size_t)o * NP + p) * 2;
                pp.dtab2[((size_t)o * 2) * NP2 + p] = d[0];
                pp.dtab2[((size_t)o * 2 + 1) * NP2 + p] = d[1];
            }
        if (sh.bw[0] < kInfH) {
            pp.nrng = pp.nrng2 = 0;
            pp.dtab.clear();
            pp.dtab2.clear();
        }
    }
    pp.pflags.assign(P, 0);
    pp.spos.assign(n, 0);
    pp.ties_heavy = nL > 0;
    for (uint32_t p = 0; p < nL; ++p) {
        uint8_t f = sh.bex[p] ? 1 : 0;
        if (sh.aex[0][p]) f |= 2;
        if (p > 0 && sh.heavy[0] < sh.light[p - 1]) f |= 4;
        pp.pflags[p] = f;
        pp.ties_heavy = pp.ties_heavy && (f & 2) && (!(f & 1) || (f & 4));
        pp.spos[sh.light[p]] = (int32_t)p;
    }
    for (uint32_t x = 0; x < H; ++x) pp.spos[sh.heavy[x]] = -1 - (int32_t)x;
    pp.hx_exist = sh.hx_exist;
    pp.hl_exist = sh.hl_exist;
    pp.hc.assign((size_t)S * 8, kInfH);
    auto wide_consts = [&](uint32_t o, const float* c) {
        for (uint32_t blk = 0; blk < pp.nblk; ++blk)
            for (uint32_t lane = 0; lane < 64; ++lane) {
                float* base = pp.tab.data() + ((((size_t)blk * S + o) * nc + sm / 2) * 64 + lane) * 4;
                for (int k = 0; k < 4; ++k) base[k] = c[k];
                if (sx) {
                    float* b2 = base + 64 * 4;
                    b2[0] = c[4];
                    b2[1] = b2[2] = b2[3] = 0.0f;
                }
            }
    };
    for (uint32_t o = 0; o < S; ++o) {
        float* c = pp.hc.data() + (size_t)o * 8;
        const float eF = hm.emis[(size_t)o * n + sh.heavy[0]];
        const float eS = H == 2 ? hm.emis[(size_t)o * n + sh.heavy[1]] : kInfH;
        c[0] = eS + (H == 2 ? sh.wh[1] : kInfH);
        c[1] = eF + sh.wh[0];
        c[2] = eS + xss;
        c[3] = eF + xff;
        c[4] = eS + xsf;
        c[5] = eF;
        c[6] = eS;
        c[7] = 0.0f;
        if (wide) wide_consts(o, c);
    }
    bool nonneg = !wide;
    for (float v : hm.val) nonneg = nonneg && v >= 0.0f;
    for (float v : hm.emis) nonneg = nonneg && v >= 0.0f;
    for (float v : hm.start) nonneg = nonneg && v >= 0.0f;
    pp.emax2 = nonneg ? 0.0f : kInfH;
    if (nonneg)
        for (uint32_t p = 0; p < nL; ++p)
            for (uint32_t o = 0; o < S; ++o) {
                const float ea = hm.emis[(size_t)o * n + sh.light[p]] + sh.aw[0][p];
                if (ea < kInfH) pp.emax2 = std::max(pp.emax2, ea);
            }
    pp.ok = true;
    return pp;
}

void DevicePipePlan::upload(const PipePlan& p, uint32_t n, uint32_t S, hipStream_t s) {
    plan = p;
    if (!p.ok) return;
    d_tab.upload(p.tab.data(), p.tab.size() * 4, s);
    d_e0.upload(p.e0.data(), p.e0.size() * 4, s);
    d_start.upload(p.start.data(), p.start.size() * 4, s);
    d_lrow.upload(p.lrow.data(), p.lrow.size() * 4, s);
    d_hc.upload(p.hc.data(), p.hc.size() * 4, s);
    d_pflags.upload(p.pflags.data(), p.pflags.size(), s);
    d_spos.upload(p.spos.data(), p.spos.size() * 4, s);
    std::memset(&view, 0, sizeof(view));
    view.pflags = d_pflags.as<uint8_t>();
    view.spos = d_spos.as<int32_t>();
    view.hx_exist = p.hx_exist;
    view.hl_exist = p.hl_exist;
    view.ties_heavy = p.ties_heavy ? 1u : 0u;
    view.tab = d_tab.as<float2>();
    view.e0 = d_e0.as<float>();
    view.start = d_start.as<float>();
    view.lrow = d_lrow.as<uint32_t>();
    view.hc = d_hc.as<float>();
    view.rowF = p.rowF;
    view.rowS = p.rowS;
    view.startF = p.startF;
    view.startS = p.startS;
    view.n = n;
    view.S = S;
    view.P = p.P;
    view.nblk = p.nblk;
    view.SM = p.SM;
    view.W = p.W;
    view.G = p.G;
    view.sx = p.sx ? 1u : 0u;
    view.wide = p.wide ? 1u : 0u;
    view.rerun = !p.wide && pipe_rerun_fits(p.P, p.W) ? 1u : 0u;
    if (p.nrng && !p.dtab.empty() && diag_lds_bytes(diag_waves_for(4), S, p.P) <= 160 * 1024) {
        d_dtab.upload(p.dtab.data(), p.dtab.size() * 4, s);
        view.dtab = d_dtab.as<float2>();
        view.nrng = p.nrng;
        if (p.nrng2 && !p.dtab2.empty() && (size_t)p.nrng2 * 128 == p.P &&
            diag_lds_bytes(diag_waves_for(4), S, p.P, 2) <= 160 * 1024) {
            d_dtab2.upload(p.dtab2.data(), p.dtab2.size() * 4, s);
            view.dtab2 = d_dtab2.as<float>();
            view.nrng2 = p.nrng2;
        }
        if (const char* e = std::getenv("SVH_DIAG_SM")) {
            const int v = std::atoi(e);
            view.dsm = v == 1 || v == 2 ? (uint32_t)v : 0u;
        }
        if (const char* e = std::getenv("SVH_DIAG_LOADER"); e && *e) view.dld = std::atoi(e) ? 2u : 1u;
    }
    view.emax2 = p.emax2;
    view.tm = !p.wide && p.SM == 2 && (p.W == 4 || (p.W == 8 && pipe_tm_supported(-8))) && S <= kPairSymbols ? 4u : 0u;
    if (const char* e = std::getenv("SVH_PIPE_TM"); e) {
        const int t = std::atoi(e);
        if (t == 0 || (t >= 1 && t <= 4 && view.tm && pipe_tm_supported(t))) view.tm = (uint32_t)t;
    }
    if (const char* e = std::getenv("SVH_PIPE_DEBUG"); e && std::atoi(e)) {
        d_stamps.alloc((size_t)65536 * kPipeStamps * 8);
        hip_check(hipMemsetAsync(d_stamps.ptr, 0, d_stamps.bytes, s), "stamps");
        view.stamps = d_stamps.as<unsigned long long>();
        view.diag = (uint32_t)std::atoi(e) >> 1;
    }
}

void DevicePipePlan::report_stamps(uint32_t nseq) const {
    if (!view.stamps) return;
    const size_t waves = (size_t)nseq * plan.G * plan.W;
    if (waves > 65536 / kPipeStamps * kPipeStamps) return;
    std::vector<unsigned long long> h(waves * kPipeStamps);
    if (hipMemcpy(h.data(), view.stamps, h.size() * 8, hipMemcpyDeviceToHost) != hipSuccess) return;
    double sum[kPipeStamps] = {}, mx[kPipeStamps] = {};
    for (size_t w = 0; w < waves; ++w)
        for (int k = 0; k < kPipeStamps; ++k) {
            sum[k] += (double)h[w * kPipeStamps + k];
            mx[k] = std::max(mx[k], (double)h[w * kPipeStamps + k]);
        }
    std::fprintf(stderr, "pipe stamps (avg / max per wave): loop %.0f/%.0f head %.0f/%.0f tail %.0f/%.0f "
                 "prev %.0f/%.0f next %.0f/%.0f gran %.0f/%.0f cons %.0f/%.0f iters %.0f slow-groups %.0f/%.0f\n",
                 sum[0] / waves, mx[0], sum[1] / waves, mx[1], sum[2] / waves, mx[2], sum[3] / waves, mx[3],
                 sum[4] / waves, mx[4], sum[5] / waves, mx[5], sum[6] / waves, mx[6], sum[7] / waves,
                 sum[14] / waves, mx[14]);
    {
        unsigned long long t0 = ~0ull, tend = 0;
        for (size_t w = 0; w < waves; ++w)
            if (h[w * kPipeStamps + 8]) {
                t0 = std::min(t0, h[w * kPipeStamps + 8]);
                tend = std::max(tend, h[w * kPipeStamps + 11]);
            }
        if (t0 != ~0ull) std::fprintf(stderr, "pipe wall (us from first entry): last sweep end %.2f\n", (tend - t0) * 0.01);
        for (uint32_t q = 0; t0 != ~0ull && q < nseq; ++q) {
            std::fprintf(stderr, "  seq %u:", q);
            for (uint32_t g = 0; g < plan.G; ++g) {
                unsigned long long en = 0, st = 0, ed = 0, tb = 0;
                for (uint32_t w = 0; w < plan.W; ++w) {
                    const unsigned long long* r = h.data() + (((size_t)q * plan.G + g) * plan.W + w) * kPipeStamps;
                    if (!r[8]) continue;
                    en = std::max(en, r[8] - t0);
                    if (w == 0) st = r[9] - t0;
                    if (w == 0 && r[13]) tb = r[13] - t0;
                    ed = std::max(ed, r[11] - t0);
                }
                const unsigned long long* r0 = h.data() + (((size_t)q * plan.G + g) * plan.W) * kPipeStamps;
                const unsigned long long hw = r0[12];
                const double mhz = r0[10] > r0[9] ? (double)r0[0] / ((double)(r0[10] - r0[9]) * 0.01) : 0.0;
                std::fprintf(stderr, " [g%u in %.1f tab %.1f st %.1f end %.1f x%u s%u c%u %.0fMHz]", g, en * 0.01, tb * 0.01,
                             st * 0.01, ed * 0.01, (unsigned)(hw >> 32) & 0xFu, (unsigned)(hw >> 13) & 0x3u,
                             (unsigned)(hw >> 8) & 0xFu, mhz);
            }
            std::fprintf(stderr, "\n");
        }
        for (size_t w = 0; t0 != ~0ull && w < waves; ++w) {
            const unsigned long long* r = h.data() + w * kPipeStamps;
            if (!r[8] || w / plan.W >= 2 * plan.G) continue;
            std::fprintf(stderr, "  wave %zu (seq-ticket %zu): entry %.2f start %.2f body_end %.2f end %.2f\n", w % plan.W,
                         w / plan.W, (r[8] - t0) * 0.01, (r[9] - t0) * 0.01, (r[10] - t0) * 0.01, (r[11] - t0) * 0.01);
        }
    }
    {
        std::fprintf(stderr, "pipe wait split by role (mean over %u rows): g w loop prev next gran cons slow\n", nseq);
        for (uint32_t g = 0; g < plan.G; ++g)
            for (uint32_t w = 0; w < plan.W; ++w) {
                double a[8] = {};
                uint32_t cnt = 0;
                for (uint32_t q = 0; q < nseq; ++q) {
                    const unsigned long long* r = h.data() + (((size_t)q * plan.G + g) * plan.W + w) * kPipeStamps;
                    if (!r[8]) continue;
                    ++cnt;
                    a[0] += (double)r[0];
                    for (int k = 3; k <= 6; ++k) a[k - 2] += (double)r[k];
                    a[5] += (double)r[14];
                }
                if (!cnt) continue;
                std::fprintf(stderr, "  role g%u w%u: %.0f %.1f %.1f %.1f %.1f %.1f\n", g, w, a[0] / cnt, a[1] / cnt,
                             a[2] / cnt, a[3] / cnt, a[4] / cnt, a[5] / cnt);
            }
    }
    uint32_t qlast = 0;
    unsigned long long elast = 0;
    for (uint32_t q = 0; q < nseq; ++q)
        for (size_t w = 0; w < (size_t)plan.G * plan.W; ++w)
            if (h[((size_t)q * plan.G * plan.W + w) * kPipeStamps + 11] > elast) {
                elast = h[((size_t)q * plan.G * plan.W + w) * kPipeStamps + 11];
                qlast = q;
            }
    for (uint32_t q : {0u, qlast}) {
        for (uint32_t g = 0; g < plan.G; ++g)
            for (uint32_t w = 0; w < plan.W; ++w) {
                const unsigned long long* r = h.data() + (((size_t)q * plan.G + g) * plan.W + w) * kPipeStamps;
                std::fprintf(stderr, "  seq %u g%u w%u: loop %llu head %llu tail %llu prev %llu next %llu gran %llu cons %llu slow %llu\n",
                             q, g, w, r[0], r[1], r[2], r[3], r[4], r[5], r[6], r[14]);
            }
        if (qlast == 0) break;
    }
}

void PipeScratchBuffers::ensure(uint32_t rows, uint32_t G, hipStream_t s) {
    if (!d_ctr.ptr) {
        d_ctr.alloc(kCtrWords * 4);
        hip_check(hipMemsetAsync(d_ctr.ptr, 0, kCtrWords * 4, s), "pipe counters");
    }
    if (view.ctr && rows <= view.rows && G <= view.G) return;
    rows = std::max(rows, view.rows);
    G = std::max(G, view.G);
    auto zeroed = [&](DeviceBuffer& d, size_t bytes) {
        d.alloc(bytes);
        hip_check(hipMemsetAsync(d.ptr, 0, d.bytes, s), "pipe scratch");
    };
    zeroed(d_done, (size_t)rows * 128);
    zeroed(d_part, (size_t)rows * G * 16);
    zeroed(d_gran, (size_t)rows * std::max<uint32_t>(G - 1, 1) * kPipeGRing * 8);
    zeroed(d_cons, (size_t)rows * G * 8);
    zeroed(d_viol, (size_t)rows * 4);
    zeroed(d_xcc, (size_t)rows * G * 4);
    view.ctr = d_ctr.as<uint32_t>();
    view.done = d_done.as<uint32_t>();
    view.part = d_part.as<uint64_t>();
    view.gran = d_gran.as<uint64_t>();
    view.cons = d_cons.as<uint32_t>();
    view.viol = d_viol.as<uint32_t>();
    view.xcc = d_xcc.as<uint32_t>();
    view.rows = rows;
    view.G = G;
}

void PipeScratchBuffers::note_launch(hipStream_t s) {
    if (launches > 0 && launches % kEpochSpan == 0) {
        hip_check(hipMemsetAsync(d_ctr.ptr, 0, d_ctr.bytes, s), "pipe epoch reset");
        hip_check(hipMemsetAsync(d_gran.ptr, 0, d_gran.bytes, s), "pipe epoch reset");
        hip_check(hipMemsetAsync(d_cons.ptr, 0, d_cons.bytes, s), "pipe epoch reset");
        hip_check(hipMemsetAsync(d_xcc.ptr, 0, d_xcc.bytes, s), "pipe epoch reset");
    }
    ++launches;
}

void DeviceBandPlan::report_stamps(uint32_t nseq) const {
    if (!(view.dbg & (4u | 128u)) || !view.stamps) return;
    std::vector<unsigned long long> h((size_t)nseq * kMaxWaves * kBandStamps);
    if (hipMemcpy(h.data(), view.stamps, h.size() * 8, hipMemcpyDeviceToHost) != hipSuccess) return;
    double sum[kBandStamps] = {};
    uint32_t cnt = 0;
    for (uint32_t q = 0; q < nseq; ++q)
        for (uint32_t w = 0; w < std::max<uint32_t>(plan.B / 64, 1); ++w, ++cnt)
// ... 269 lines not shown
        for (uint32_t k = 0; k < nt; ++k) {
            sp.thr[t + k] = h;
            sp.tcp[t + k] = n * sp.KL + cpoff[h];
        }
        t += nt;
    }
    sp.amax.assign(H, 0.0f);
    bool nonneg = true;
    for (uint32_t j = 0; j < n; ++j)
        for (uint32_t e = hm.rowptr[j]; e < hm.rowptr[j + 1]; ++e) {
            nonneg = nonneg && hm.val[e] >= 0.0f;
            const int32_t h = hid[hm.col[e]];
            if (h < 0) continue;
            for (uint32_t o = 0; o < S; ++o) {
                const float a = hm.emis[(size_t)o * n + j] + hm.val[e];
                if (a < kInfH) sp.amax[h] = std::max(sp.amax[h], a);
            }
        }
    for (float e : hm.emis) nonneg = nonneg && e >= 0.0f;
    for (float e : hm.start) nonneg = nonneg && e >= 0.0f;
    sp.prune = nonneg;
    if (H == 0) {
        sp.hrow.push_back(0);
        sp.amax.push_back(0.0f);
    }
    sp.ok = true;
    return sp;
}

void DeviceSpec2Plan::upload(const Spec2Plan& p, const HostModel& hm, const float* d_emis, hipStream_t s) {
    plan = p;
    std::memset(&view, 0, sizeof(view));
    if (!p.ok) return;
    d_la.upload(p.la.data(), p.la.size() * 4, s);
    d_lb.upload(p.lb.data(), p.lb.size() * 4, s);
    d_lv.upload(p.lv.data(), p.lv.size() * 4, s);
    d_thr.upload(p.thr.data(), p.thr.size() * 4, s);
    d_tcp.upload(p.tcp.data(), p.tcp.size() * 4, s);
    d_ha.upload(p.ha.data(), p.ha.size() * 4, s);
    d_hb.upload(p.hb.data(), p.hb.size() * 4, s);
    d_hv.upload(p.hv.data(), p.hv.size() * 4, s);
    d_hrow.upload(p.hrow.data(), p.hrow.size() * 4, s);
    d_amax.upload(p.amax.data(), p.amax.size() * 4, s);
    view.emis = d_emis;
    view.la = d_la.as<uint32_t>();
    view.lb = d_lb.as<uint32_t>();
    view.lv = d_lv.as<float>();
    view.thr = d_thr.as<uint32_t>();
    view.tcp = d_tcp.as<uint32_t>();
    view.ha = d_ha.as<uint32_t>();
    view.hb = d_hb.as<uint32_t>();
    view.hv = d_hv.as<float>();
    view.hrow = d_hrow.as<uint32_t>();
    view.amax = d_amax.as<float>();
    view.n = hm.n;
    view.S = hm.S;
    view.H = p.H;
    view.NP = p.NP;
    view.R = p.R;
    view.KL = p.KL;
    view.NHS = p.NHS;
    view.nhs = p.nhs;
    view.prune = p.prune ? 1u : 0u;
    if (const char* e = std::getenv("SVH_SPEC2_DEBUG"); e && std::atoi(e)) {
        d_stamps.alloc((size_t)4096 * 16 * kSpec2Stamps * 8);
        hip_check(hipMemsetAsync(d_stamps.ptr, 0, d_stamps.bytes, s), "stamps");
        view.stamps = d_stamps.as<unsigned long long>();
    }
}

void DeviceSpec2Plan::report_stamps(uint32_t nseq) const {
    if (!view.stamps) return;
    nseq = std::min<uint32_t>(nseq, 4096);
    std::vector<unsigned long long> h((size_t)nseq * 16 * kSpec2Stamps);
    if (hipMemcpy(h.data(), view.stamps, h.size() * 8, hipMemcpyDeviceToHost) != hipSuccess) return;
    double sum[kSpec2Stamps] = {};
    double chunks = 0;
    for (uint32_t q = 0; q < nseq; ++q)
        for (uint32_t w = 0; w < 16; ++w) {
            const unsigned long long* r = h.data() + ((size_t)q * 16 + w) * kSpec2Stamps;
            for (int k = 0; k < 7; ++k) sum[k] += (double)r[k];
            chunks += (double)r[7];
        }
    if (chunks <= 0) return;
    std::fprintf(stderr, "spec2 cycles per chunk and wave (s_memtime): phase1 %.0f bar1 %.0f phase1b %.0f bar2 %.0f "
                         "phase2 %.0f bar3 %.0f loop %.0f (%.0f chunks x waves)\n",
                 sum[0] / chunks, sum[1] / chunks, sum[2] / chunks, sum[3] / chunks, sum[4] / chunks, sum[5] / chunks,
                 sum[6] / chunks, chunks);
}

void Model::spec_build(uint32_t level, hipStream_t s) {
    std::lock_guard<std::mutex> lock(mu);
    DeviceGuard g(device);
    if (!s) s = stream;
    d_products = DeviceBuffer();
    spec_level = 0;
    spec2_on = false;
    if (level <= 1) {
        spec_level = level;
        return;
    }
    static const bool dense_env = std::getenv("SVH_SPEC_DENSE") && std::atoi(std::getenv("SVH_SPEC_DENSE")) == 1;
    if (level == 2 && !dense_env && !spec_dense) {
        if (!spec2.plan.ok) {
            const Spec2Plan sp = make_spec2_plan(host);
            if (sp.ok) {
                spec2.upload(sp, host, d_gemis.as<float>(), s);
                hip_check(hipStreamSynchronize(s), "spec2 plan upload");
            }
        }
        if (spec2.plan.ok) {
            spec2_on = true;
            spec_level = level;
            return;
        }
    }
    const CsrModel c = csr_view();
    if (host.n > 65535) throw Error(SVH_E_UNSUPPORTED, "_spec level >= 2 needs states_num <= 65535");
    pstride = (host.n + 3) & ~3u;
    const uint64_t mat = (uint64_t)host.n * pstride;
    uint64_t keys = host.S;
    for (uint32_t l = 2; l <= level; ++l) {
        keys *= host.S;
        if (keys / host.S > 65535 / ((host.S + 31) / 32))
            throw Error(SVH_E_UNSUPPORTED, "_spec level too high for the precompute grid");
    }
    const uint64_t final_bytes = keys * mat * 4;
    const uint64_t prev_bytes = (keys / host.S) * mat * 4;
    size_t free_b = 0, total_b = 0;
    hip_check(hipMemGetInfo(&free_b, &total_b), "hipMemGetInfo");
    if (final_bytes + prev_bytes + (64ull << 20) > free_b)
        throw Error(SVH_E_NOMEM, "_spec products need " + std::to_string(final_bytes + prev_bytes) +
                                     " bytes of HBM, " + std::to_string(free_b) + " free");
    d_mfold.alloc((size_t)host.nnz() * host.S * 4);
    hip_check(launch_spec_fold(c, d_mfold.as<float>(), s), "spec fold");
    DeviceBuffer prev;
    prev.alloc((size_t)host.S * mat * 4);
    hip_check(launch_spec_densify(c, d_mfold.as<float>(), prev.as<float>(), pstride, s), "spec densify");
    uint64_t kprev = host.S;
    for (uint32_t l = 2; l <= level; ++l) {
        DeviceBuffer next;
        next.alloc((size_t)(kprev * host.S * mat * 4));
        hip_check(launch_spec_extend(c, d_mfold.as<float>(), prev.as<float>(), kprev,
                                     next.as<float>(), pstride, s),
                  "spec extend");
        hip_check(hipStreamSynchronize(s), "spec extend");
        prev = std::move(next);
        kprev *= host.S;
    }
    d_products = std::move(prev);
    spec_level = level;
}

svh_model_info Model::info(uint32_t nseq, bool paths, uint32_t level) const {
    svh_model_info i;
    std::memset(&i, 0, sizeof(i));
    const bool steps = level <= 1 || spec_level < 2;
    const bool pq = paths && steps;
    const PassPlan pl = resolve(nseq, pq, level, nseq != 0 && pq == paths);
    const StepKernel named = level >= 2 ? pl.no_diag : pl.step;
    const DevicePlan* p = fused_plan(pq);
    i.kernel = kernel_id(named);
    i.family = p ? p->plan.family : -1;
    i.threads = p ? (int32_t)p->plan.B : (int32_t)std::min<uint32_t>(1024, round_up(host.n, 64));
    i.slots = p ? (int32_t)p->plan.SM : 0;
    i.light_terms = p ? (int32_t)p->plan.R : 0;
    i.heavy_rows = p ? (int32_t)p->plan.H : 0;
    i.heavy_uniform = (p && p->plan.mode == kHeavyUniform) ? 1 : 0;
    i.device = device;
    i.n = host.n;
    i.S = host.S;
    i.nnz = host.nnz();
    i.lds_bytes = p ? p->plan.lds_bytes : generic_lds_bytes(host.n);
    if (const DeviceBandPlan* bpl = band_plan(pl)) {
        i.threads = (int32_t)bpl->plan.B;
        i.slots = (int32_t)bpl->plan.SM;
        i.light_terms = (int32_t)bpl->plan.HA + 1;
        i.heavy_rows = (int32_t)bpl->plan.H;
        i.heavy_uniform = 1;
        i.lds_bytes = bpl->plan.chain ? chain_lds_bytes() : bpl->plan.lds_bytes;
    }
    i.spec_level = spec_level;
    i.spec_bytes = d_products.bytes;
    i.paths_kernel = kernel_id(resolve(1, true, 0, true).step);
    const bool wide_chain = band_wide.plan.ok && on_band(resolve(0, false, 0, false).step);
    i.wide_threads = wide_chain ? (int32_t)band_wide.plan.B : 0;
    i.wide_slots = wide_chain ? (int32_t)band_wide.plan.SM : 0;
    i.cu_count = cu_count;
    if (pipelined(named)) {
        const DevicePipePlan& ppl = named == StepKernel::PipeWide ? pipe_wide : pipe;
        uint32_t w = ppl.plan.wide ? pipew_waves_for(ppl.view, nseq) : ppl.plan.W;
        if (ppl.plan.wide && paths) w = std::min(w, pipew_paths_waves_max(ppl.plan.SM, host.S, ppl.plan.sx));
        i.threads = (int32_t)(64 * w);
        i.slots = (int32_t)ppl.plan.SM;
        i.lds_bytes = ppl.plan.wide ? pipew_lds_bytes(ppl.plan.SM, w, host.S, ppl.plan.sx, paths)
                                    : pipe_lds_bytes(ppl.plan.W, host.S);
    }
    const ReportedThresholds t = reported_thresholds(caps);
    if (pipe_wide.plan.ok) {
        i.pipew_slots = (int32_t)pipe_wide.plan.SM;
        i.pipew_waves = (int32_t)pipe_wide.plan.W;
        i.pipew_blocks = (int32_t)pipe_wide.plan.G;
    }
    if (pipe.plan.ok) {
        i.pipe_slots = (int32_t)pipe.plan.SM;
        i.pipe_waves = (int32_t)pipe.plan.W;
        i.pipe_groups = (int32_t)pipe.plan.G;
    }
    if (pipe.view.dtab) i.diag_ranges = (int32_t)pipe.plan.nrng;
    i.pipe_max_nseq = t.pipe_max_nseq;
    i.pipe_max_nseq_paths = t.pipe_max_nseq_paths;
    i.pipew_min_nseq = t.pipew_min_nseq;
    i.diag_max_nseq = t.diag_max_nseq;
    if (pl.step == StepKernel::Diag && level <= 1) {
        const uint32_t w = diag_waves_for(nseq);
        i.threads = (int32_t)(64 * w);
        i.slots = 1;
        if (!pq) {
            i.diag_sm = (int32_t)diag_sm_for(pipe.view, nseq, false, false);
            i.lds_bytes = diag_lds_bytes(w, host.S, pipe.plan.P, (uint32_t)i.diag_sm, diag_loader_for(pipe.view, nseq, false, false));
        } else {
            i.diag_sm = 1;
            i.lds_bytes = diag_paths_lds_bytes(w, host.S, pipe.plan.sx);
        }
    } else if (pl.step == StepKernel::Diag && !pq) {
        i.diag_sm = (int32_t)diag_sm_for(pipe.view, nseq, true, false);
    }
    if (nseq && pl.chunks == ChunkRoute::Spec2Pipe) {
        i.kernel = SVH_KERNEL_SPEC2_PIPE;
        i.threads = (int32_t)(64 * pipe.plan.W);
        i.slots = (int32_t)pipe.plan.SM;
        i.lds_bytes = pipe_lds_bytes(pipe.plan.W, host.S);
        i.spec_bytes = 0;
    } else if (nseq && pl.chunks == ChunkRoute::Spec2Diag) {
        const uint32_t w = diag_waves_for(nseq);
        i.kernel = SVH_KERNEL_SPEC2_DIAG;
        i.threads = (int32_t)(64 * w);
        i.slots = 1;
        i.lds_bytes = diag_l2_lds_bytes(w, host.S);
        i.spec_bytes = 0;
    } else if (nseq && pl.chunks == ChunkRoute::Spec2) {
        const Spec2Plan& sp = spec2.plan;
        i.kernel = SVH_KERNEL_SPEC2;
        i.threads = (int32_t)kSpec2Threads;
        i.slots = 0;
        i.light_terms = (int32_t)sp.KL;
        i.heavy_rows = (int32_t)sp.H;
        i.lds_bytes = spec2_lds_layout(host.n, sp.KL, sp.NP, sp.H).bytes;
        i.spec_bytes = spec2.d_la.bytes + spec2.d_lb.bytes + spec2.d_lv.bytes + spec2.d_thr.bytes + spec2.d_tcp.bytes +
                       spec2.d_ha.bytes + spec2.d_hb.bytes + spec2.d_hv.bytes + spec2.d_hrow.bytes + spec2.d_amax.bytes;
    }
    return i;
}

Batch::Batch(Model* m, uint64_t nseq_, const uint64_t* offs, const uint64_t* symbols, uint32_t flags)
    : model(m) {
    init(flags);
    load(nseq_, offs, symbols, nullptr, m->stream);
    hip_check(hipStreamSynchronize(m->stream), "batch upload");
}

Batch::Batch(Model* m, uint64_t nseq_, const uint64_t* offs, const uint8_t* symbols, uint32_t flags)
    : model(m) {
    init(flags);
    load(nseq_, offs, nullptr, symbols, m->stream);
    hip_check(hipStreamSynchronize(m->stream), "batch upload");
}

void Batch::init(uint32_t flags) {
    paths = (flags & SVH_BATCH_PATHS) != 0;
    if (paths && model->resolve(1, true, 0, true).records == PathRecords::Backpointers && model->host.n >= kNoPred)
        throw Error(SVH_E_UNSUPPORTED, "paths need states_num < 65535 for models the chain kernel does not cover");
    timing = (flags & SVH_BATCH_NO_TIMING) == 0;
    DeviceGuard g(model->device);
    if (timing) {
        hip_check(hipEventCreate(&ev_start), "hipEventCreate");
        hip_check(hipEventCreate(&ev_stop), "hipEventCreate");
    }
}

void Batch::load(uint64_t nseq_, const uint64_t* offs, const uint64_t* sym64, const uint8_t* sym8,
                 hipStream_t s, const uint64_t* const* seqp) {
    if (nseq_ == 0) throw Error(SVH_E_INVALID, "empty batch");
    if (nseq_ > 0x7FFFFFFFull) throw Error(SVH_E_UNSUPPORTED, "too many sequences in one batch");
    if (!offs || (!sym64 && !sym8 && !seqp)) throw Error(SVH_E_INVALID, "null offsets/symbols");
    if (seqp)
        for (uint64_t q = 0; q < nseq_; ++q)
            if (!seqp[q] && offs[q + 1] > offs[q]) throw Error(SVH_E_INVALID, "null sequence pointer");
    nseq = (uint32_t)nseq_;
    plan = model->resolve(nseq, paths, 0, true);
    chain_paths = paths && plan.records != PathRecords::Backpointers;
    pipe_paths = plan.records == PathRecords::Pipe;
    diag_paths = plan.records == PathRecords::Diag;
    const DeviceBandPlan* cpl = chain_paths ? model->band_plan(plan) : nullptr;
    const DevicePipePlan* ppl = pipe_paths ? &model->pipe_plan(plan) : nullptr;
    const DevicePipePlan* dpl = diag_paths ? &model->pipe_plan(plan) : nullptr;
    const bool recs = pipe_paths || diag_paths;
    offsets.assign(offs, offs + nseq + 1);
    lens.resize(nseq);
    h_symoff.resize(nseq);
    h_pathoff.resize(nseq);
    h_bpoff.resize(nseq);
    h_cmoff.resize(nseq);
    h_hroff.resize(nseq);
    h_ckoff.resize(nseq);
    h_pmoff.resize(recs ? nseq : 0);
    h_proff.resize(recs ? nseq : 0);
    h_pcoff.resize(recs ? nseq : 0);
    h_fcoff.resize(recs ? nseq : 0);
    h_dcoff.resize(diag_paths ? nseq : 0);
    uint64_t bytes = 0, bpn = 0, cmn = 0, hrn = 0, ckn = 0, pmn = 0, prn = 0, pcn = 0, fcn = 0, dcn = 0;
    for (uint32_t q = 0; q < nseq; ++q) {
        if (offs[q + 1] < offs[q]) throw Error(SVH_E_INVALID, "offsets must be non-decreasing");
        const uint64_t len = offs[q + 1] - offs[q];
        if (len == 0)
            throw Error(SVH_E_INVALID, "empty observation sequence (reference: seq[0] is undefined)");
        if (len > 0xFFFFFF00ull) throw Error(SVH_E_UNSUPPORTED, "sequence too long");
        lens[q] = (uint32_t)len;
        h_symoff[q] = bytes;
        bytes += ((len + kSymPad + 4 + 15) / 16) * 16;
        if (cpl) {
            h_cmoff[q] = cmn;
            cmn += chain_mask_words(len, cpl->plan.B / 64, cpl->plan.SM);
            h_hroff[q] = hrn;
            hrn += chain_hrec_words(len);
            h_ckoff[q] = ckn;
            ckn += chain_ckpt_floats(len, cpl->plan.SM, cpl->plan.B);
            if (ppl) {
                h_pmoff[q] = pmn;
                pmn += pipe_mask_words(len, ppl->plan.nblk, ppl->plan.SM);
                h_proff[q] = prn;
                prn += pipe_prec_count(len, ppl->plan.nblk, pipe_prec_parts(ppl->plan.wide));
                h_pcoff[q] = pcn;
                pcn += pipe_ckpt_floats(len, ppl->plan.P);
                h_fcoff[q] = fcn;
                fcn += pipe_fck_floats(len);
            } else if (dpl) {
                const uint32_t nr = dpl->plan.nrng;
                h_pmoff[q] = pmn;
                pmn += diag_mask_words(len, nr);
                h_proff[q] = prn;
                prn += diag_mu_floats(len, nr);
                h_pcoff[q] = pcn;
                pcn += diag_ckpt_floats(len, nr);
                h_fcoff[q] = fcn;
                fcn += pipe_fck_floats(len);
                h_dcoff[q] = dcn;
                dcn += diag_cck_floats(len, nr);
            }
        } else if (paths) {
            h_bpoff[q] = bpn;
            bpn += (len - 1) * (uint64_t)model->host.n;
        }
        h_pathoff[q] = offs[q] - offs[0];
    }
    total = offs[nseq] - offs[0];
    DeviceGuard g(model->device);
    struct Section {
        size_t off = 0, bytes = 0;
    };
    size_t in_bytes = 0;
    auto section = [&](size_t nb) {
        Section x;
        x.off = in_bytes;
        x.bytes = nb;
        in_bytes += (nb + 15) & ~(size_t)15;
        return x;
    };
    const Section s_sym = section(bytes), s_symoff = section((size_t)nseq * 8), s_begin = section((size_t)nseq * 4),
                  s_end = section((size_t)nseq * 4);
    const bool cp = paths && chain_paths, pp = cp && recs, dgp = cp && diag_paths, fp = paths && !chain_paths;
    const Section s_path = section(paths ? (size_t)nseq * 8 : 0), s_cm = section(cp ? (size_t)nseq * 8 : 0),
                  s_hr = section(cp ? (size_t)nseq * 8 : 0), s_ck = section(cp ? (size_t)nseq * 8 : 0),
// ... 756 lines not shown
```

spec_viterbi_amd/csrc/runtime.h:

```cpp
#pragma once

#include <hip/hip_runtime.h>

#include <algorithm>
#include <cstdint>
#include <memory>
#include <mutex>
#include <stdexcept>
#include <string>
#include <vector>

#include "dispatch.h"
#include "error.h"
#include "kernels.h"
#include "set_table.h"
#include "svh.h"

namespace svh {


void hip_check(hipError_t e, const char* what);

struct DeviceGuard {
    int prev = -1;
    explicit DeviceGuard(int dev);
    ~DeviceGuard();
};

struct DeviceBuffer {
    void* ptr = nullptr;
    size_t bytes = 0;
    DeviceBuffer() = default;
    DeviceBuffer(const DeviceBuffer&) = delete;
    DeviceBuffer& operator=(const DeviceBuffer&) = delete;
    DeviceBuffer(DeviceBuffer&& o) noexcept : ptr(o.ptr), bytes(o.bytes) { o.ptr = nullptr; o.bytes = 0; }
    DeviceBuffer& operator=(DeviceBuffer&& o) noexcept;
    ~DeviceBuffer();
    void alloc(size_t nbytes);
    void upload(const void* src, size_t nbytes, hipStream_t s);
    void reserve(size_t nbytes);
    void upload_async(const void* src, size_t nbytes, hipStream_t s);
    template <class T> T* as() const { return static_cast<T*>(ptr); }
};

struct HostModel {
    uint32_t n = 0, S = 0;
    std::vector<float> start;
    std::vector<float> emis;
    std::vector<uint32_t> rowptr;
    std::vector<uint32_t> col;
    std::vector<float> val;
    uint32_t nnz() const { return (uint32_t)col.size(); }
};

HostModel build_host_model(uint64_t n, uint64_t S, uint64_t nstart, const uint64_t* start_cols,
                           const float* start_vals, const float* emissions, uint64_t ntrans,
                           const uint64_t* src, const uint64_t* dst, const float* prob);

struct Plan {
    bool fused = false;
    int family = -1;
    uint32_t B = 0, SM = 0, R = 0, HM = 0, XM = 0, H = 0;
    int mode = kHeavyGeneral;
    uint32_t estride = 0, vstride = 0;
    int hrow[kMaxHeavy] = {0, 0, 0, 0};
    float hw[kMaxHeavy] = {0, 0, 0, 0};
    uint32_t xk[kMaxHeavy][kMaxExc] = {};
    float xw[kMaxHeavy][kMaxExc] = {};
    std::vector<uint32_t> lcol;
    std::vector<float> lval;
    std::vector<float> hval;
    std::vector<uint8_t> hvalid;
    std::vector<float> hmask;
    std::vector<float> emis_pad;
    std::vector<float> start_pad;
    size_t lds_bytes = 0;
};

Plan make_plan(const HostModel& hm, int max_threads, bool allow_uniform);

struct DevicePlan {
    Plan plan;
    DeviceBuffer d_emis, d_start, d_lcol, d_lval, d_hval, d_hvalid, d_hmask;
    FusedModel view{};
    void upload(const Plan& p, hipStream_t s);
};

struct BandPlan {
    bool ok = false;
    bool chain = false;
    bool ge = false;
    uint32_t B = 0, SM = 0, HA = 0, H = 0, nL = 0, erow = 0;
    int hrow[kBandHeavy] = {0, 0};
    int hvalid[kBandHeavy] = {0, 0};
    float hstart[kBandHeavy] = {0, 0};
    std::vector<float> erows, erows_t, start, aw, bw;
    std::vector<uint32_t> lrow;
    std::vector<uint8_t> pflags;
    std::vector<int32_t> spos;
    uint32_t hx_exist = 0, hl_exist = 0;
    bool ties_heavy = false;
    size_t lds_bytes = 0;
    bool paths_ok() const { return ok && chain && !ge && HA <= 1 && chain_paths_supported((int)SM, (int)(B / 64)); }
};
BandPlan make_band_plan(const HostModel& hm, int max_threads, bool chain, int ge_waves = -1);

struct DeviceBandPlan {
    BandPlan plan;
    DeviceBuffer d_erows, d_erows_t, d_start, d_aw, d_bw, d_lrow, d_stamps, d_pflags, d_spos;
    BandModel view{};
    void upload(const BandPlan& p, uint32_t n, uint32_t S, hipStream_t s);
    void report_stamps(uint32_t nseq) const;
};

struct PipePlan {
    bool ok = false;
    bool sx = false;
    uint32_t SM = 0, W = 0, G = 0, nblk = 0, P = 0;
    int rowF = -1, rowS = -1;
    float startF = 0, startS = 0;
    std::vector<float> tab;
    std::vector<float> e0;
    std::vector<float> start;
    std::vector<uint32_t> lrow;
    std::vector<float> hc;
    bool wide = false;
    std::vector<float> dtab;
    uint32_t nrng = 0;
    std::vector<float> dtab2;
    uint32_t nrng2 = 0;
    float emax2 = 0.0f;
    std::vector<uint8_t> pflags;
    std::vector<int32_t> spos;
    uint32_t hx_exist = 0, hl_exist = 0;
    bool ties_heavy = false;
};
PipePlan make_pipe_plan(const HostModel& hm, uint32_t sm = 0, uint32_t waves = 0, bool wide = false);

struct DevicePipePlan {
    PipePlan plan;
    DeviceBuffer d_tab, d_e0, d_start, d_lrow, d_hc, d_stamps, d_pflags, d_spos, d_dtab, d_dtab2;
    PipeModel view{};
    void upload(const PipePlan& p, uint32_t n, uint32_t S, hipStream_t s);
    void report_stamps(uint32_t nseq) const;
};

struct Spec2Plan {
    bool ok = false;
    bool prune = false;
    uint32_t R = 0, KL = 0, NHS = 0, nhs = 0, H = 0, NP = 0;
    std::vector<uint32_t> la, lb, thr, tcp, ha, hb, hrow;
    std::vector<float> lv, hv, amax;
};
Spec2Plan make_spec2_plan(const HostModel& hm);

struct DeviceSpec2Plan {
    Spec2Plan plan;
    DeviceBuffer d_la, d_lb, d_lv, d_thr, d_tcp, d_ha, d_hb, d_hv, d_hrow, d_amax, d_stamps;
    Spec2Model view{};
    void report_stamps(uint32_t nseq) const;
    void upload(const Spec2Plan& p, const HostModel& hm, const float* d_emis, hipStream_t s);
};

template <class T>
struct Pinned {
    T* p = nullptr;
    size_t n = 0;
    Pinned() = default;
    Pinned(const Pinned&) = delete;
    Pinned& operator=(const Pinned&) = delete;
    ~Pinned() {
        if (p) (void)hipHostFree(p);
    }
    T* reserve(size_t count) {
        if (count > n) {
            if (p) (void)hipHostFree(p);
            p = nullptr;
            n = 0;
            hip_check(hipHostMalloc((void**)&p, std::max<size_t>(count, 1) * sizeof(T), hipHostMallocDefault),
                      "hipHostMalloc");
            n = count;
        }
        return p;
    }
};

struct PipeScratchBuffers {
    DeviceBuffer d_ctr, d_done, d_part, d_gran, d_cons, d_viol, d_xcc;
    PipeScratch view{};
    uint64_t launches = 0;
    void ensure(uint32_t rows, uint32_t G, hipStream_t s);
    void note_launch(hipStream_t s);
    static constexpr uint64_t kEpochSpan = 1ull << 19;
};

struct Model {
    std::mutex mu;
    int device = 0;
    ModelCaps caps;
    HostModel host;
    hipStream_t stream = nullptr;
    DeviceBandPlan band;
    DeviceBandPlan band_wide;
    uint32_t cu_count = 0;
    DevicePipePlan pipe;
    DevicePipePlan pipe_wide;
    DevicePlan fast_plan;
    DevicePlan paths_plan_storage;
    const DevicePlan* paths_plan = nullptr;
    DeviceBuffer d_gemis, d_gstart, d_rowptr, d_col, d_val, d_rowof;
    uint32_t spec_level = 0;
    uint32_t pstride = 0;
    DeviceBuffer d_mfold, d_products;
    DeviceSpec2Plan spec2;
    bool spec2_on = false;
    bool spec_dense = false;

    Model(const HostModel& h, const svh_model_opts* opts);
    ~Model();
    CsrModel csr_view() const;
    PassPlan resolve(uint32_t rows, bool paths, uint32_t level, bool scratch) const;
    const DeviceBandPlan* band_plan(const PassPlan& p) const;
    const DevicePipePlan& pipe_plan(const PassPlan& p) const { return p.step == StepKernel::PipeWide ? pipe_wide : pipe; }
    const DevicePlan* fused_plan(bool paths) const;
    void spec_build(uint32_t level, hipStream_t s);
    svh_model_info info(uint32_t nseq = 0, bool paths = false, uint32_t level = 0) const;
    void launch_steps(const FusedBatch& b, const PassPlan& p, hipStream_t s) const;
};

struct Batch {
    Model* model;
    uint32_t nseq = 0;
    bool paths = false;
    PassPlan plan;
    std::vector<uint64_t> offsets;
    std::vector<uint32_t> lens;
    uint64_t total = 0;
    DeviceBuffer d_in;
    Pinned<uint8_t> h_in;
    uint8_t* p_sym = nullptr;
    uint64_t* p_symoff = nullptr;
    uint32_t *p_begin = nullptr, *p_end = nullptr;
    uint64_t *p_pathoff = nullptr, *p_cmoff = nullptr, *p_hroff = nullptr, *p_ckoff = nullptr, *p_pmoff = nullptr,
             *p_proff = nullptr, *p_pcoff = nullptr, *p_fcoff = nullptr, *p_dcoff = nullptr, *p_bpoff = nullptr;
    DeviceBuffer d_out;
    uint32_t* p_fault = nullptr;
    int64_t* p_best = nullptr;
    float* p_scores = nullptr;
    DeviceBuffer d_bp, d_paths;
    bool chain_paths = false;
    DeviceBuffer d_cmask, d_hrec, d_ckpt;
    bool pipe_paths = false;
    DeviceBuffer d_pmask, d_prec, d_pck, d_fck;
    bool diag_paths = false;
    DeviceBuffer d_dcc;
    PipeScratchBuffers pipe;

    DeviceBuffer d_vbuf, d_nchunks, d_tbegin, d_vrow;
    DeviceBuffer d_l2viol;
    bool l2_ran = false;
    uint32_t spec_ready_level = 0;
    uint32_t max_chunks = 0;
    hipEvent_t ev_start = nullptr, ev_stop = nullptr;
    bool timing = true;
    hipStream_t last_stream = nullptr;
    bool ran = false;
    hipStream_t set_stream = nullptr;
    hipStream_t own_stream() const { return set_stream ? set_stream : model->stream; }

    Pinned<uint8_t> h_out;
    std::vector<uint64_t> h_symoff, h_pathoff, h_bpoff, h_cmoff, h_hroff, h_ckoff;
    std::vector<uint64_t> h_pmoff, h_proff, h_pcoff, h_fcoff, h_dcoff;

    Batch(Model* m, uint64_t nseq, const uint64_t* offsets, const uint64_t* symbols, uint32_t flags);
    Batch(Model* m, uint64_t nseq, const uint64_t* offsets, const uint8_t* symbols, uint32_t flags);
    void load(uint64_t nseq, const uint64_t* offsets, const uint64_t* sym64, const uint8_t* sym8, hipStream_t s,
              const uint64_t* const* seqp = nullptr);
    ~Batch();
    void run(uint32_t level, hipStream_t s);
    void read(hipStream_t s, float* scores, int64_t* best, int32_t* paths);
    float elapsed_ms();
    float step_floor_ms(hipStream_t s, uint32_t reps);
    PipeScratchBuffers floor_scratch;
    DeviceBuffer d_floor_out;
    uint64_t pipe_fallbacks(uint32_t* rows = nullptr);
    bool pipe_ran = false;
    void run_time_parallel(uint32_t seg, uint32_t probe, float tol, hipStream_t s, uint64_t* fallbacks);
    void read_async(hipStream_t s, float* scores, int64_t* best, int32_t* paths);
    void check_fault(hipStream_t s);
    void inject_fault(hipStream_t s);

    void begin_set_run(hipStream_t s, DiagSetEntry* e);
    const DevicePipePlan* set_plan() const;

  private:
    void init(uint32_t flags);
    void report_fault(uint32_t f, hipStream_t s);
    FusedBatch scores_view() const;
};

struct BatchSet {
    std::mutex mu;
    std::vector<std::unique_ptr<Batch>> members;
    std::vector<uint8_t> grouped;
    int device = 0;
    uint32_t nseq = 0, cus = 0;
    bool timing = true;
    SetTable table;
    std::vector<DiagSetEntry> h_entries;
    DeviceBuffer d_entries, d_first;
    DiagSetLaunch launch{};
    uint64_t last_launches = 0;
    hipEvent_t ev_start = nullptr, ev_stop = nullptr;
    bool ran = false;

    BatchSet(Model* const* models, uint64_t nmodels, uint64_t nseq, const uint64_t* offsets, const uint8_t* symbols,
             uint32_t flags);
    ~BatchSet();
    void run(uint32_t level, hipStream_t s);
    svh_batchset_info info();
    float elapsed_ms();

  private:
    void refresh(hipStream_t s);
};

}
```

spec_viterbi_amd/csrc/svh_api.cpp:

```cpp
#include <chrono>
#include <cstdio>
#include <cstdlib>
#include <fstream>
#include <memory>
#include <mutex>
#include <new>
#include <string>

#include "HMM.h"
#include "data_reader.h"
#include "runtime.h"
#include "stream.h"
#include "svh.h"

struct svh_hmm {
    HMM hmm;
};
struct svh_ess {
    HMM::Emit_seq_vec_t seqs;
};
struct svh_model {
    std::unique_ptr<svh::Model> impl;
    std::mutex oneshot_mu;
    std::unique_ptr<svh::Batch> oneshot[2];
// ... 143 lines not shown
void svh_ess_free(svh_ess_t e) { delete e; }

int svh_model_create(uint64_t n, uint64_t S, uint64_t nstart, const uint64_t* start_cols,
                     const float* start_vals, const float* emissions, uint64_t ntrans,
                     const uint64_t* trans_src, const uint64_t* trans_dst,
                     const float* trans_prob, const svh_model_opts* opts, svh_model_t* out) {
    return guarded([&] {
        require(out != nullptr, "null output handle");
        *out = nullptr;
        svh::HostModel h = svh::build_host_model(n, S, nstart, start_cols, start_vals, emissions,
                                                 ntrans, trans_src, trans_dst, trans_prob);
        auto m = std::make_unique<svh_model>();
        m->impl = std::make_unique<svh::Model>(h, opts);
        *out = m.release();
    });
}

int svh_model_destroy(svh_model_t m) {
    return guarded([&] { delete m; });
}

int svh_model_get_info(svh_model_t m, svh_model_info* info) {
    return guarded([&] {
        require(m && info, "null argument");
        *info = m->impl->info();
    });
}

int svh_spec_build(svh_model_t m, uint32_t level, void* stream) {
    return guarded([&] {
        require(m != nullptr, "null model");
        m->impl->spec_build(level, static_cast<hipStream_t>(stream));
    });
}

int svh_batch_create(svh_model_t m, uint64_t nseq, const uint64_t* offsets,
                     const uint64_t* symbols, uint32_t flags, svh_batch_t* out) {
    return guarded([&] {
        require(m && out, "null argument");
        *out = nullptr;
        auto b = std::make_unique<svh_batch>();
        b->owner = m;
        b->impl = std::make_unique<svh::Batch>(m->impl.get(), nseq, offsets, symbols, flags);
        *out = b.release();
    });
}

int svh_batch_create_u8(svh_model_t m, uint64_t nseq, const uint64_t* offsets, const uint8_t* symbols,
                        uint32_t flags, svh_batch_t* out) {
    return guarded([&] {
        require(m && out, "null argument");
        *out = nullptr;
        auto b = std::make_unique<svh_batch>();
        b->owner = m;
        b->impl = std::make_unique<svh::Batch>(m->impl.get(), nseq, offsets, symbols, flags);
        *out = b.release();
    });
}

int svh_batch_run(svh_batch_t b, uint32_t level, void* stream) {
    return guarded([&] {
        require(b != nullptr, "null batch");
        b->get()->run(level, static_cast<hipStream_t>(stream));
    });
}

int svh_batch_run_time_parallel(svh_batch_t b, uint32_t seg_len, uint32_t probe_len, float rel_tol,
                                void* stream, uint64_t* fallbacks) {
    return guarded([&] {
        require(b != nullptr, "null batch");
        b->get()->run_time_parallel(seg_len, probe_len, rel_tol, static_cast<hipStream_t>(stream), fallbacks);
    });
}

int svh_host_alloc(size_t bytes, void** out) {
    return guarded([&] {
        require(out != nullptr, "null argument");
        *out = nullptr;
        svh::hip_check(hipHostMalloc(out, bytes ? bytes : 1, hipHostMallocDefault), "hipHostMalloc");
    });
}

int svh_host_free(void* p) {
    return guarded([&] {
        if (p) svh::hip_check(hipHostFree(p), "hipHostFree");
    });
}

int svh_batch_read(svh_batch_t b, void* stream, float* scores, int64_t* best_state,
                   int32_t* paths) {
    return guarded([&] {
        require(b != nullptr, "null batch");
        b->get()->read(static_cast<hipStream_t>(stream), scores, best_state, paths);
    });
}

int svh_batch_device_results(svh_batch_t b, float** scores, int64_t** best_state) {
    return guarded([&] {
        require(b != nullptr, "null batch");
        if (scores) *scores = b->get()->p_scores;
        if (best_state) *best_state = b->get()->p_best;
    });
}

int svh_batch_elapsed_ms(svh_batch_t b, float* ms) {
    return guarded([&] {
        require(b && ms, "null argument");
        *ms = b->get()->elapsed_ms();
    });
}

int svh_batch_step_floor_ms(svh_batch_t b, void* stream, uint32_t reps, float* ms) {
    return guarded([&] {
        require(b && ms && reps > 0, "null argument or reps == 0");
        *ms = b->get()->step_floor_ms(static_cast<hipStream_t>(stream), reps);
    });
}

int svh_batch_fallback_rows(svh_batch_t b, uint32_t* flags) {
    return guarded([&] {
        require(b && flags, "null argument");
        (void)b->get()->pipe_fallbacks(flags);
    });
}

int svh_batch_fallbacks(svh_batch_t b, uint64_t* rows) {
    return guarded([&] {
        require(b && rows, "null argument");
        *rows = b->get()->pipe_fallbacks();
    });
}

int svh_pipe_variant_built(int32_t slots, int32_t waves, int32_t table_mode, int32_t* built) {
    return guarded([&] {
        require(built != nullptr, "null argument");
        bool ok = false;
        if (table_mode == 0) ok = svh::pipe_supported(slots, waves, false);
        else ok = slots == 2 && waves == 4 && svh::pipe_tm_supported(table_mode);
        *built = ok ? 1 : 0;
    });
}

int svh_batch_debug_fault(svh_batch_t b, void* stream) {
    return guarded([&] {
        require(b != nullptr, "null batch");
        b->get()->inject_fault(static_cast<hipStream_t>(stream));
    });
}

int svh_batch_plan(svh_batch_t b, uint32_t level, svh_model_info* info) {
    return guarded([&] {
        require(b && info, "null argument");
        *info = b->get()->model->info(b->get()->nseq, b->get()->paths, level);
    });
}

int svh_batch_destroy(svh_batch_t b) {
    return guarded([&] {
        if (b && b->view) throw svh::Error(SVH_E_INVALID, "a set's member is destroyed with its set (svh_batchset_destroy)");
        delete b;
    });
}

int svh_batchset_create(const svh_model_t* models, uint64_t nmodels, uint64_t nseq, const uint64_t* offsets,
                        const uint8_t* symbols, uint32_t flags, svh_batchset_t* out) {
    return guarded([&] {
        require(models && out, "null argument");
        *out = nullptr;
        std::vector<svh::Model*> ms(nmodels);
        for (uint64_t i = 0; i < nmodels; ++i) {
            require(models[i] != nullptr, "null model");
            ms[i] = models[i]->impl.get();
        }
        auto s = std::make_unique<svh_batchset>();
        s->impl = std::make_unique<svh::BatchSet>(ms.data(), nmodels, nseq, offsets, symbols, flags);
        for (uint64_t i = 0; i < nmodels; ++i) {
            auto v = std::make_unique<svh_batch>();
            v->owner = models[i];
            v->view = s->impl->members[i].get();
            s->views.push_back(std::move(v));
        }
        *out = s.release();
    });
}

int svh_batchset_run(svh_batchset_t s, uint32_t level, void* stream) {
    return guarded([&] {
        require(s != nullptr, "null batch set");
        s->impl->run(level, static_cast<hipStream_t>(stream));
    });
}

int svh_batchset_member(svh_batchset_t s, uint64_t i, svh_batch_t* out) {
    return guarded([&] {
        require(s && out, "null argument");
        *out = nullptr;
        if (i >= s->views.size()) throw svh::Error(SVH_E_RANGE, "batch set: member index out of range");
        *out = s->views[i].get();
    });
}

int svh_batchset_get_info(svh_batchset_t s, svh_batchset_info* info) {
    return guarded([&] {
        require(s && info, "null argument");
        *info = s->impl->info();
    });
}

int svh_batchset_elapsed_ms(svh_batchset_t s, float* ms) {
    return guarded([&] {
        require(s && ms, "null argument");
        *ms = s->impl->elapsed_ms();
    });
}

int svh_batchset_destroy(svh_batchset_t s) {
    return guarded([&] { delete s; });
}

namespace {
void oneshot(svh_model_t m, uint32_t level, uint64_t nseq, const uint64_t* offsets, const uint64_t* sym64,
             const uint8_t* sym8, const uint64_t* const* seqp, float* scores, int64_t* best_state, int32_t* paths) {
    require(m != nullptr, "null model");
    require(offsets && (sym64 || sym8 || seqp), "null offsets/symbols");
    std::lock_guard<std::mutex> lock(m->oneshot_mu);
    std::unique_ptr<svh::Batch>& b = m->oneshot[paths ? 1 : 0];
    if (!b) {
        static const uint64_t one[2] = {0, 1};
        static const uint8_t zero = 0;
        b = std::make_unique<svh::Batch>(m->impl.get(), 1, one, &zero, paths ? SVH_BATCH_PATHS : 0u);
    }
    static const bool trace = std::getenv("SVH_TRACE_ONESHOT") && std::atoi(std::getenv("SVH_TRACE_ONESHOT"));
    if (!trace) {
        b->load(nseq, offsets, sym64, sym8, m->impl->stream, seqp);
        b->run(level, nullptr);
        b->read(nullptr, scores, best_state, paths);
        return;
    }
    using clk = std::chrono::steady_clock;
    hipEvent_t e0;
    (void)hipEventCreate(&e0);
    const auto t0 = clk::now();
    (void)hipEventRecord(e0, m->impl->stream);
    b->load(nseq, offsets, sym64, sym8, m->impl->stream, seqp);
    const auto t1 = clk::now();
    b->run(level, nullptr);
    const auto t2 = clk::now();
    b->read(nullptr, scores, best_state, paths);
    const auto t3 = clk::now();
    float upload_ms = 0.0f, kernel_ms = 0.0f;
    (void)hipEventElapsedTime(&upload_ms, e0, b->ev_start);
    (void)hipEventElapsedTime(&kernel_ms, b->ev_start, b->ev_stop);
    (void)hipEventDestroy(e0);
    auto us = [](clk::time_point a, clk::time_point c) { return std::chrono::duration<double, std::micro>(c - a).count(); };
    std::fprintf(stderr, "oneshot trace (us): load %.1f run-enqueue %.1f read %.1f total %.1f | gpu: upload-to-run-start %.1f "
                 "run %.1f\n", us(t0, t1), us(t1, t2), us(t2, t3), us(t0, t3), upload_ms * 1e3, kernel_ms * 1e3);
}
}

int svh_viterbi(svh_model_t m, uint32_t level, uint64_t nseq, const uint64_t* offsets,
                const uint64_t* symbols, float* scores, int64_t* best_state, int32_t* paths) {
    return guarded([&] { oneshot(m, level, nseq, offsets, symbols, nullptr, nullptr, scores, best_state, paths); });
}

int svh_viterbi_u8(svh_model_t m, uint32_t level, uint64_t nseq, const uint64_t* offsets,
                   const uint8_t* symbols, float* scores, int64_t* best_state, int32_t* paths) {
    return guarded([&] { oneshot(m, level, nseq, offsets, nullptr, symbols, nullptr, scores, best_state, paths); });
}

int svh_viterbi_seqs(svh_model_t m, uint32_t level, uint64_t nseq, const uint64_t* const* seqs,
                     const uint64_t* lens, float* scores, int64_t* best_state, int32_t* paths) {
    return guarded([&] {
        require(seqs && lens, "null sequences/lengths");
        std::vector<uint64_t> offs(nseq + 1, 0);
        for (uint64_t q = 0; q < nseq; ++q) offs[q + 1] = offs[q] + lens[q];
        oneshot(m, level, nseq, offs.data(), nullptr, nullptr, seqs, scores, best_state, paths);
    });
}

int svh_reader_open(const char* path, int format, svh_reader_t* out) {
    return guarded([&] {
        require(path && out, "null argument");
        *out = nullptr;
        auto r = std::make_unique<svh_reader>();
        r->impl = std::make_unique<svh::SeqReader>(path, format);
        *out = r.release();
    });
}

int svh_reader_next(svh_reader_t r, uint64_t max_seqs, uint64_t max_symbols, uint64_t* nseq,
                    const uint64_t** offsets, const uint8_t** symbols) {
    return guarded([&] {
        require(r && nseq, "null argument");
        *nseq = 0;
        if (!r->impl->next(max_seqs, max_symbols, r->offsets, r->symbols)) r->offsets.assign(1, 0);
        *nseq = r->offsets.size() - 1;
        if (offsets) *offsets = r->offsets.data();
        if (symbols) *symbols = r->symbols.data();
    });
}

void svh_reader_close(svh_reader_t r) { delete r; }

int svh_decode_file(svh_model_t m, const char* path, int format, uint32_t level, uint32_t flags,
                    uint64_t max_seqs, uint64_t max_symbols, svh_result_fn fn, void* user,
                    uint64_t* nseq_total) {
// ... 10 lines not shown
```

spec_viterbi_amd/viterbi.py:

```python
from __future__ import annotations

import abc
import ctypes
import hashlib

import numpy as np

from . import _lib
from .hmm import HMM, pack_sequences

_u64 = ctypes.POINTER(ctypes.c_uint64)
_f32 = ctypes.POINTER(ctypes.c_float)
_i64 = ctypes.POINTER(ctypes.c_int64)
_i32 = ctypes.POINTER(ctypes.c_int32)
_u32 = ctypes.POINTER(ctypes.c_uint32)


def _p(a, t):
    return a.ctypes.data_as(t)


def pinned_empty(shape, dtype=np.float32) -> np.ndarray:
    import weakref

    dtype = np.dtype(dtype)
    n = int(np.prod(shape)) * dtype.itemsize
    ptr = ctypes.c_void_p()
    _lib.check(_lib.lib.svh_host_alloc(max(n, 1), ctypes.byref(ptr)))
    buf = (ctypes.c_uint8 * max(n, 1)).from_address(ptr.value)
    arr = np.frombuffer(buf, np.uint8, count=n).view(dtype).reshape(shape)
    weakref.finalize(buf, _lib.lib.svh_host_free, ptr.value)
    return arr


def _result_arrays(out, nseq: int, n: int):
    if out is None:
        return np.empty((nseq, n), np.float32), np.empty(nseq, np.int64)
    scores, best = out
    if (scores.shape != (nseq, n) or scores.dtype != np.float32 or not scores.flags.c_contiguous
            or best.shape != (nseq,) or best.dtype != np.int64 or not best.flags.c_contiguous):
        raise ValueError("out: (float32 [nseq, n], int64 [nseq]) C-contiguous arrays expected")
    return scores, best


class DeviceModel:

    def __init__(self, hmm: HMM, device: int = -1, kernel: int = _lib.SVH_KERNEL_AUTO, max_threads: int = 0,
                 flags: int = 0):
        self.n = int(hmm.states_num)
        self.S = int(hmm.emit_num)
        opts = _lib.svh_model_opts(device, kernel, max_threads, flags)
        h = ctypes.c_void_p()
        sc = np.ascontiguousarray(hmm.start_probabilities_cols, np.uint64)
        sv = np.ascontiguousarray(hmm.start_probabilities, np.float32)
        em = np.ascontiguousarray(hmm.emissions, np.float32)
        src = np.ascontiguousarray(hmm.trans_rows, np.uint64)
        dst = np.ascontiguousarray(hmm.trans_cols, np.uint64)
        pr = np.ascontiguousarray(hmm.trans_probs, np.float32)
        _lib.check(_lib.lib.svh_model_create(self.n, self.S, sc.size, _p(sc, _u64), _p(sv, _f32), _p(em, _f32),
                                             pr.size, _p(src, _u64), _p(dst, _u64), _p(pr, _f32),
                                             ctypes.byref(opts), ctypes.byref(h)))
        self._h = h

    @property
    def handle(self):
        return self._h

    def info(self) -> dict:
        i = _lib.svh_model_info()
        _lib.check(_lib.lib.svh_model_get_info(self._h, ctypes.byref(i)))
        return {name: getattr(i, name) for name, _ in i._fields_}

    def spec_build(self, level: int, stream: int | None = None) -> None:
        _lib.check(_lib.lib.svh_spec_build(self._h, int(level), ctypes.c_void_p(stream or 0)))

    def batch(self, seqs, paths: bool = False, timing: bool = True) -> "DeviceBatch":
        return DeviceBatch(self, seqs, paths, timing)

    def viterbi(self, seqs, level: int = 0, paths: bool = False):
        seqs = [s if isinstance(s, np.ndarray) and s.dtype == np.uint64 and s.flags.c_contiguous
                else np.ascontiguousarray(s, np.uint64) for s in seqs]
        nseq = len(seqs)
        lens = np.fromiter((s.size for s in seqs), np.uint64, nseq)
        ptrs = np.fromiter((s.ctypes.data for s in seqs), np.uint64, nseq)
        scores = np.empty((nseq, self.n), np.float32)
        best = np.empty(nseq, np.int64)
        pth = np.empty(int(lens.sum()), np.int32) if paths else None
        _lib.check(_lib.lib.svh_viterbi_seqs(self._h, int(level), nseq, _p(ptrs, _u64), _p(lens, _u64),
                                             _p(scores, _f32), _p(best, _i64), _p(pth, _i32) if paths else None))
        if paths:
            offsets = np.zeros(nseq + 1, np.int64)
            np.cumsum(lens, out=offsets[1:])
            return scores, best, [pth[offsets[q]:offsets[q + 1]] for q in range(nseq)]
        return scores, best

    def viterbi_packed(self, offsets, symbols, level: int = 0, paths: bool = False, out=None):
        offsets = np.ascontiguousarray(offsets, np.uint64)
        symbols = np.asarray(symbols)
        if offsets.ndim != 1 or offsets.size < 1:
            raise ValueError("offsets: a 1-D array of nseq + 1 entries expected")
        if symbols.ndim != 1:
            raise ValueError("symbols: a 1-D array expected")
        if np.any(offsets[1:] < offsets[:-1]) or int(offsets[-1]) > symbols.size:
            raise ValueError("offsets must be non-decreasing with offsets[-1] <= symbols.size")
        nseq = offsets.size - 1
        scores, best = _result_arrays(out, nseq, self.n)
        pth = np.empty(int(offsets[-1] - offsets[0]) if nseq else 0, np.int32) if paths else None
        if symbols.dtype == np.uint8:
            symbols = np.ascontiguousarray(symbols)
            fn, sp = _lib.lib.svh_viterbi_u8, _p(symbols, ctypes.POINTER(ctypes.c_uint8))
        else:
            symbols = np.ascontiguousarray(symbols, np.uint64)
            fn, sp = _lib.lib.svh_viterbi, _p(symbols, _u64)
        _lib.check(fn(self._h, int(level), nseq, _p(offsets, _u64), sp, _p(scores, _f32), _p(best, _i64),
                      _p(pth, _i32) if paths else None))
        if paths:
            base = int(offsets[0])
            return scores, best, [pth[int(offsets[q]) - base:int(offsets[q + 1]) - base] for q in range(nseq)]
        return scores, best

    def close(self):
        if getattr(self, "_h", None):
            _lib.lib.svh_model_destroy(self._h)
            self._h = None

    def __del__(self):
        try:
            self.close()
        except Exception:
            pass


class DeviceBatch:

    def __init__(self, model: DeviceModel, seqs, paths: bool = False, timing: bool = True):
        self.model = model
        self.offsets, symbols = pack_sequences(seqs)
        self.nseq = self.offsets.size - 1
        self.paths = paths
        self.total = int(self.offsets[-1])
        h = ctypes.c_void_p()
        _lib.check(_lib.lib.svh_batch_create(model.handle, self.nseq, _p(self.offsets, _u64), _p(symbols, _u64),
                                             (_lib.SVH_BATCH_PATHS if paths else 0) |
                                             (0 if timing else _lib.SVH_BATCH_NO_TIMING), ctypes.byref(h)))
        self._h = h

    def run(self, level: int = 0, stream: int | None = None) -> None:
        _lib.check(_lib.lib.svh_batch_run(self._h, int(level), ctypes.c_void_p(stream or 0)))

    def run_time_parallel(self, seg_len: int = 1024, probe_len: int = 256, rel_tol: float = 1e-6,
                          stream: int | None = None) -> int:
        fb = ctypes.c_uint64()
        _lib.check(_lib.lib.svh_batch_run_time_parallel(self._h, int(seg_len), int(probe_len), float(rel_tol),
                                                         ctypes.c_void_p(stream or 0), ctypes.byref(fb)))
        return int(fb.value)

    def read(self, stream: int | None = None, want_paths: bool = False, out=None):
        scores, best = _result_arrays(out, self.nseq, self.model.n)
        pth = np.empty(self.total, np.int32) if want_paths else None
        _lib.check(_lib.lib.svh_batch_read(self._h, ctypes.c_void_p(stream or 0), _p(scores, _f32), _p(best, _i64),
                                           _p(pth, _i32) if want_paths else None))
        if want_paths:
            return scores, best, [pth[self.offsets[q]:self.offsets[q + 1]] for q in range(self.nseq)]
        return scores, best

    def device_results(self) -> tuple[int, int]:
        s, b = ctypes.c_void_p(), ctypes.c_void_p()
        _lib.check(_lib.lib.svh_batch_device_results(self._h, ctypes.byref(s), ctypes.byref(b)))
        return int(s.value or 0), int(b.value or 0)

    def plan(self, level: int = 0) -> dict:
        i = _lib.svh_model_info()
        _lib.check(_lib.lib.svh_batch_plan(self._h, int(level), ctypes.byref(i)))
        return {name: getattr(i, name) for name, _ in i._fields_}

    def fallbacks(self) -> int:
        r = ctypes.c_uint64()
        _lib.check(_lib.lib.svh_batch_fallbacks(self._h, ctypes.byref(r)))
        return int(r.value)

    def fallback_rows(self) -> np.ndarray:
        f = np.zeros(self.nseq, np.uint32)
        _lib.check(_lib.lib.svh_batch_fallback_rows(self._h, _p(f, _u32)))
        return f

    def debug_fault(self, stream: int | None = None) -> None:
        _lib.check(_lib.lib.svh_batch_debug_fault(self._h, ctypes.c_void_p(stream or 0)))

    def step_floor_ms(self, reps: int = 10, stream: int | None = None) -> float:
        ms = ctypes.c_float()
        _lib.check(_lib.lib.svh_batch_step_floor_ms(self._h, ctypes.c_void_p(stream or 0), int(reps), ctypes.byref(ms)))
        return float(ms.value)

    def elapsed_ms(self) -> float:
        ms = ctypes.c_float()
        _lib.check(_lib.lib.svh_batch_elapsed_ms(self._h, ctypes.byref(ms)))
        return float(ms.value)

    def close(self):
        if getattr(self, "_h", None):
            if not getattr(self, "_borrowed", False):
                _lib.lib.svh_batch_destroy(self._h)
            self._h = None

    def __del__(self):
        try:
            self.close()
        except Exception:
            pass


class DeviceModelSet:

    def __init__(self, models):
        self.models = list(models)
        if not self.models:
            raise ValueError("DeviceModelSet: no models")

    def batch(self, seqs, timing: bool = True) -> "DeviceBatchSet":
        return DeviceBatchSet(self, seqs, timing)


class DeviceBatchSet:

    def __init__(self, mset: DeviceModelSet, seqs, timing: bool = True, paths: bool = False):
        self.mset = mset
        self.offsets, sym64 = pack_sequences(seqs)
        self.nseq = self.offsets.size - 1
        if sym64.size and int(sym64.max()) > 255:
            raise _lib.SvhError(_lib.SVH_E_RANGE, f"symbol {int(sym64.max())} out of range (a set takes 8-bit symbols)")
        symbols = np.ascontiguousarray(sym64, np.uint8)
        handles = (ctypes.c_void_p * len(mset.models))(*[m.handle for m in mset.models])
        h = ctypes.c_void_p()
        _lib.check(_lib.lib.svh_batchset_create(handles, len(mset.models), self.nseq, _p(self.offsets, _u64),
                                                _p(symbols, ctypes.POINTER(ctypes.c_uint8)),
                                                (0 if timing else _lib.SVH_BATCH_NO_TIMING) |
                                                (_lib.SVH_BATCH_PATHS if paths else 0), ctypes.byref(h)))
        self._h = h
        self.members = []
        for i, model in enumerate(mset.models):
            bh = ctypes.c_void_p()
            _lib.check(_lib.lib.svh_batchset_member(self._h, i, ctypes.byref(bh)))
            b = DeviceBatch.__new__(DeviceBatch)
            b.model, b.offsets, b.nseq, b.paths, b.total = model, self.offsets, self.nseq, False, int(self.offsets[-1])
            b._h, b._borrowed = bh, True
            self.members.append(b)

    def run(self, level: int = 0, stream: int | None = None) -> None:
        _lib.check(_lib.lib.svh_batchset_run(self._h, int(level), ctypes.c_void_p(stream or 0)))

    def read(self, stream: int | None = None) -> list:
        return [b.read(stream) for b in self.members]

    def info(self) -> dict:
        i = _lib.svh_batchset_info()
        _lib.check(_lib.lib.svh_batchset_get_info(self._h, ctypes.byref(i)))
        return {name: getattr(i, name) for name, _ in i._fields_}

    def elapsed_ms(self) -> float:
        ms = ctypes.c_float()
        _lib.check(_lib.lib.svh_batchset_elapsed_ms(self._h, ctypes.byref(ms)))
        return float(ms.value)

    def close(self):
        if getattr(self, "_h", None):
            for b in self.members:
                b._h = None
            _lib.lib.svh_batchset_destroy(self._h)
            self._h = None

    def __del__(self):
        try:
            self.close()
        except Exception:
            pass


class Viterbi_impl(abc.ABC):

    @abc.abstractmethod
    def run_Viterbi(self, hmm: HMM, seq) -> np.ndarray:
        ...


class Viterbi_spec_impl(abc.ABC):

    def __init__(self, level: int):
        self.level = int(level)

    @abc.abstractmethod
    def spec_with(self, hmm: HMM) -> None:
        ...

    @abc.abstractmethod
    def run_Viterbi_spec(self, seq) -> np.ndarray:
        ...

    def get_level(self) -> int:
        return self.level


def hmm_fingerprint(hmm: HMM) -> bytes:
    h = hashlib.blake2b(digest_size=16)
    h.update(np.array([hmm.states_num, hmm.emit_num], np.uint64).tobytes())
    for a in (hmm.trans_rows, hmm.trans_cols, hmm.trans_probs, hmm.emissions, hmm.start_probabilities_cols,
              hmm.start_probabilities):
        a = np.ascontiguousarray(a)
        h.update(np.array([a.size], np.uint64).tobytes())
        h.update(a.tobytes())
    return h.digest()


class HIP_impl(Viterbi_impl):

    def __init__(self, device: int = -1, **model_opts):
        self.device = device
        self.model_opts = model_opts
        self._cache: tuple[bytes, DeviceModel] | None = None

    def _model(self, hmm: HMM) -> DeviceModel:
        key = hmm_fingerprint(hmm)
        if self._cache is None or self._cache[0] != key:
            if self._cache is not None:
                self._cache[1].close()
            self._cache = (key, DeviceModel(hmm, self.device, **self.model_opts))
        return self._cache[1]

# ... 30 lines not shown
```

Measured before the change: 3.247 million M state-updates/s.

## Add quad-interleaved emission table ring for two-diagonal diag kernel

Adds a host-built float4 emission table that packs each lane's four DM=2 emission values (two diagonals, two symbols) contiguously, plus an LDS ring layout that holds them. The kernel fills the ring with 16-byte LDS DMA (or vector stores) from the loader wave and reads all four values with one ds_read_b128, where it previously issued four scalar LDS loads. It adjusts the waitcnt accounting to match. The cost is a larger LDS ring and an extra device table. The path is used only when the two-diagonal loader mode is selected and the ring fits in 160 KB.

```diff
diff --git a/include/svh.h b/include/svh.h
--- a/include/svh.h
+++ b/include/svh.h
@@ -108,6 +108,7 @@
 int svh_batch_elapsed_ms(svh_batch_t b, float* ms);
 int svh_batch_step_floor_ms(svh_batch_t b, void* stream, uint32_t reps, float* ms);
 int svh_batch_plan(svh_batch_t b, uint32_t level, svh_model_info* info);
+int svh_batch_diag_quad(svh_batch_t b, uint32_t level, int32_t* quad, uint64_t* lds_bytes);
 int svh_batch_fallbacks(svh_batch_t b, uint64_t* rows);
 int svh_batch_fallback_rows(svh_batch_t b, uint32_t* flags);
 int svh_pipe_variant_built(int32_t slots, int32_t waves, int32_t table_mode, int32_t* built);
diff --git a/spec_viterbi_amd/_lib.py b/spec_viterbi_amd/_lib.py
--- a/spec_viterbi_amd/_lib.py
+++ b/spec_viterbi_amd/_lib.py
@@ -100,6 +100,7 @@
     "svh_batch_fallback_rows": (c_int, [c_void_p, P_u32]),
     "svh_batch_plan": (c_int, [c_void_p, c_uint32, POINTER(svh_model_info)]),
     "svh_batch_fallbacks": (c_int, [c_void_p, P_u64]),
+    "svh_batch_diag_quad": (c_int, [c_void_p, c_uint32, POINTER(c_int32), P_u64]),
     "svh_pipe_variant_built": (c_int, [ctypes.c_int32, ctypes.c_int32, ctypes.c_int32, POINTER(ctypes.c_int32)]),
     "svh_batch_debug_fault": (c_int, [c_void_p, c_void_p]),
     "svh_batch_destroy": (c_int, [c_void_p]),
diff --git a/spec_viterbi_amd/csrc/diag.hip b/spec_viterbi_amd/csrc/diag.hip
--- a/spec_viterbi_amd/csrc/diag.hip
+++ b/spec_viterbi_amd/csrc/diag.hip
@@ -55,6 +55,9 @@
 #ifndef SVH_DIAG_LDDRAIN
 #define SVH_DIAG_LDDRAIN 1
 #endif
+#ifndef SVH_DIAG_QDMA
+#define SVH_DIAG_QDMA 1
+#endif
 #ifndef SVH_DIAG_DONE_STRIDE
 #define SVH_DIAG_DONE_STRIDE 1
 #endif
@@ -64,6 +67,10 @@
 }
 __device__ __forceinline__ float lds_ld1(uint32_t a) {
     return *(const __attribute__((address_space(3))) float*)(size_t)a;
+}
+typedef float f4 __attribute__((ext_vector_type(4)));
+__device__ __forceinline__ f4 lds_ld4(uint32_t a) {
+    return *(const __attribute__((address_space(3))) f4*)(size_t)a;
 }
 
 __device__ __forceinline__ void check_off(float a, float b) {
@@ -80,8 +87,9 @@
     __builtin_amdgcn_sched_barrier(0);
 }
 
-__host__ __device__ constexpr size_t diag_lds_main(uint32_t W, uint32_t S, bool sx, uint32_t dm = 1, bool ld = false) {
-    return ((size_t)S * (dm == 2 ? kDRS2 : kDRS) * 2 + (size_t)S * 8 + (size_t)W * (ld ? 3 : 2) * kDK * (kDE + 1 + (sx ? 1 : 0)) + 2 * W) * 4;
+__host__ __device__ constexpr size_t diag_lds_main(uint32_t W, uint32_t S, bool sx, uint32_t dm = 1, bool ld = false,
+                                                   bool quad = false) {
+    return ((size_t)S * (quad ? kDRS * 2 : dm == 2 ? kDRS2 : kDRS) * 2 + (size_t)S * 8 + (size_t)W * (ld ? 3 : 2) * kDK * (kDE + 1 + (sx ? 1 : 0)) + 2 * W) * 4;
 }
 
 constexpr uint32_t kFS = 8;
@@ -90,7 +98,7 @@
     return ((diag_lds_main(W, S, sx) + 15) & ~(size_t)15) + (size_t)W * kFS * 64 * 4;
 }
 
-template <int W, bool SX, bool PATHS = false, int DM = 1, bool LD = false, bool FL = false>
+template <int W, bool SX, bool PATHS = false, int DM = 1, bool LD = false, bool FL = false, bool QD = false>
 __global__ __launch_bounds__(64 * (W + (LD ? 1 : 0))) __attribute__((amdgpu_waves_per_eu(2)))
 void diag_viterbi_kernel(PipeModel m, FusedBatch b, PipeScratch x) {
     const uint32_t bx = blockIdx.x;
@@ -110,7 +118,7 @@
 template <int W>
 __global__ __launch_bounds__(64 * W) __attribute__((amdgpu_waves_per_eu(2)))
 void diag_set_kernel(const DiagSetEntry* __restrict__ e, const uint32_t* __restrict__ first, uint32_t ne) {
-    constexpr bool SX = false, PATHS = false, LD = false, FL = false;
+    constexpr bool SX = false, PATHS = false, LD = false, FL = false, QD = false;
     constexpr int DM = 1;
     const uint32_t lane = threadIdx.x & 63u, gbx = blockIdx.x;
     uint32_t cnt = 0;
@@ -125,7 +133,8 @@
     const uint32_t i = (uint32_t)uniform((int)(cnt - 1));
     const uint32_t f0 = first[i];
     DiagSetEntry ent = e[i];
-    in_global(ent.m.tab, ent.m.e0, ent.m.start, ent.m.lrow, ent.m.hc, ent.m.dtab, ent.m.pflags, ent.m.spos, ent.m.stamps, ent.m.dtab2);
+    in_global(ent.m.tab, ent.m.e0, ent.m.start, ent.m.lrow, ent.m.hc, ent.m.dtab, ent.m.pflags, ent.m.spos, ent.m.stamps, ent.m.dtab2,
+              ent.m.dtab4);
     in_global(ent.b.symbols, ent.b.sym_off, ent.b.begin, ent.b.end, ent.b.v_in, ent.b.v_in_row, ent.b.scores, ent.b.best,
               ent.b.run_mask, ent.b.fault);
     in_global(ent.x.ctr, ent.x.done, ent.x.part, ent.x.gran, ent.x.cons, ent.x.viol, ent.x.xcc);
@@ -186,6 +195,15 @@
                   : reinterpret_cast<const void*>(&diag_viterbi_kernel<W, false, false, DM, true>);
     }
 }
+template <int W>
+const void* diag_quad_ptr(bool sx) {
+    if constexpr (SVH_DIAG_AB != 0 || SVH_DIAG_FINISH != 0 || kDK != 64) {
+        return nullptr;
+    } else {
+        return sx ? reinterpret_cast<const void*>(&diag_viterbi_kernel<W, true, false, 2, true, false, true>)
+                  : reinterpret_cast<const void*>(&diag_viterbi_kernel<W, false, false, 2, true, false, true>);
+    }
+}
 template <int DM>
 const void* diag_floor_ptr(bool sx) {
     if constexpr (SVH_DIAG_AB != 0 || SVH_DIAG_FINISH != 0) {
@@ -205,13 +223,15 @@
 
 uint32_t diag_waves_for(uint64_t nseq) { return nseq >= 4 ? 4u : nseq >= 2 ? 2u : 1u; }
 
-static size_t diag_lds(uint32_t W, uint32_t S, uint32_t P, bool sx, uint32_t dm = 1, bool ld = false) {
+static size_t diag_lds(uint32_t W, uint32_t S, uint32_t P, bool sx, uint32_t dm = 1, bool ld = false, bool quad = false) {
     const size_t rerun = (2 * (size_t)P + 2 * W) * 4;
-    const size_t mainb = diag_lds_main(W, S, sx, dm, ld);
+    const size_t mainb = diag_lds_main(W, S, sx, dm, ld, quad);
     return mainb > rerun ? mainb : rerun;
 }
 
-size_t diag_lds_bytes(uint32_t W, uint32_t S, uint32_t P, uint32_t dm, bool ld) { return diag_lds(W, S, P, true, dm, ld); }
+size_t diag_lds_bytes(uint32_t W, uint32_t S, uint32_t P, uint32_t dm, bool ld, bool quad) {
+    return diag_lds(W, S, P, true, dm, ld, quad);
+}
 
 uint32_t diag_sm_for(const PipeModel& m, uint64_t nseq, bool resumed, bool paths) {
     if (paths || !m.dtab2 || !m.nrng2 || SVH_DIAG_AB != 0 || SVH_DIAG_FINISH != 0) return 1;
@@ -229,6 +249,16 @@
     if (m.dld == 3) return W == 4;
     if (m.dld == 2) return true;
     return m.cus && (nseq + W - 1) / W * (dm == 2 ? m.nrng2 : m.nrng) <= m.cus;
+}
+
+bool diag_quad_table_fits(uint32_t S, uint32_t P, bool sx) {
+    return SVH_DIAG_AB == 0 && SVH_DIAG_FINISH == 0 && kDK == 64 && diag_lds(1, S, P, sx, 2, true, true) <= 160 * 1024;
+}
+
+bool diag_quad_for(const PipeModel& m, uint64_t nseq, bool resumed, bool paths) {
+    if (!m.dtab4 || m.dqd == 1 || m.dld == 3 || SVH_DIAG_AB != 0 || SVH_DIAG_FINISH != 0 || kDK != 64) return false;
+    if (diag_sm_for(m, nseq, resumed, paths) != 2 || !diag_loader_for(m, nseq, resumed, paths)) return false;
+    return diag_lds(diag_waves_for(nseq), m.S, m.P, m.sx != 0, 2, true, true) <= 160 * 1024;
 }
 
 size_t diag_paths_lds_bytes(uint32_t W, uint32_t S, bool sx) { return diag_lds_paths(W, S, sx); }
@@ -252,14 +282,16 @@
     if (dm == 2 && ((size_t)m.nrng2 * 128 != m.P || x.G < m.nrng2)) return hipErrorInvalidValue;
     const bool sx = m.sx != 0;
     const bool ld = diag_loader_for(m, b.nseq, b.v_in != nullptr, paths);
+    const bool quad = diag_quad_for(m, b.nseq, b.v_in != nullptr, paths);
     const void* fn = paths     ? (W == 4 ? diag_paths_ptr<4>() : W == 2 ? diag_paths_ptr<2>() : diag_paths_ptr<1>())
                      : ld && m.dld == 3 ? (dm == 2 ? diag_floor_ptr<2>(sx) : diag_floor_ptr<1>(sx))
+                     : quad    ? (W == 4 ? diag_quad_ptr<4>(sx) : W == 2 ? diag_quad_ptr<2>(sx) : diag_quad_ptr<1>(sx))
                      : ld      ? (dm == 2 ? (W == 4 ? diag_loader_ptr<4, 2>(sx) : W == 2 ? diag_loader_ptr<2, 2>(sx) : diag_loader_ptr<1, 2>(sx))
                                           : (W == 4 ? diag_loader_ptr<4, 1>(sx) : W == 2 ? diag_loader_ptr<2, 1>(sx) : diag_loader_ptr<1, 1>(sx)))
                      : dm == 2 ? (W == 4 ? diag_ptr<4, 2>(sx) : W == 2 ? diag_ptr<2, 2>(sx) : diag_ptr<1, 2>(sx))
                                : (W == 4 ? diag_ptr<4>(sx) : W == 2 ? diag_ptr<2>(sx) : diag_ptr<1>(sx));
-    size_t lds = paths ? diag_lds_paths(W, m.S, sx) : diag_lds(W, m.S, m.P, sx, dm, ld);
-    if (lds > 160 * 1024) return hipErrorInvalidValue;
+    size_t lds = paths ? diag_lds_paths(W, m.S, sx) : diag_lds(W, m.S, m.P, sx, dm, ld, quad);
+    if (lds > 160 * 1024 || !fn) return hipErrorInvalidValue;
     const uint64_t grid = ((uint64_t)b.nseq + W - 1) / W * (dm == 2 ? m.nrng2 : m.nrng);
     if (grid > 0x7FFFFFFFull) return hipErrorInvalidValue;
     if (m.cus) {
diff --git a/spec_viterbi_amd/csrc/diag_body.h b/spec_viterbi_amd/csrc/diag_body.h
--- a/spec_viterbi_amd/csrc/diag_body.h
+++ b/spec_viterbi_amd/csrc/diag_body.h
@@ -1,10 +1,12 @@
     static_assert(DM == 1 || (DM == 2 && !PATHS), "decoded paths keep one diagonal per lane");
     static_assert(!LD || (!PATHS && SVH_DIAG_AB == 0 && SVH_DIAG_FINISH == 0), "the loader wave: scores only");
     static_assert(!FL || LD, "the floor is a loader-wave launch");
+    static_assert(!QD || (DM == 2 && LD && !PATHS && !FL && kDK == 64),
+                  "the quad ring: two diagonals per lane, the loader wave, scores only; a group is one wave's 64 x 16 bytes");
     constexpr uint32_t NB = LD ? 3 : 2;
     extern __shared__ __attribute__((aligned(16))) float lds[];
     constexpr uint32_t RW = 64 * DM;
-    constexpr uint32_t RS = DM == 2 ? kDRS2 : kDRS;
+    constexpr uint32_t RS = QD ? kDRS * 2 : DM == 2 ? kDRS2 : kDRS;
     const uint32_t S = m.S, NR = DM == 2 ? m.nrng2 : m.nrng, NP = NR * RW, P = m.P;
     float* ring = lds;
     float* hcr = ring + (size_t)S * RS * 2;
@@ -147,7 +149,7 @@
     auto sbuildl = [&](uint32_t kb) {
         if (lane < kDK) {
             const uint32_t i = kb * kDK + 1 + lane;
-            const uint32_t ro = (i % kDR) * (DM == 2 ? 4u : 8u);
+            const uint32_t ro = (i % kDR) * (QD ? 16u : DM == 2 ? 4u : 8u);
             const uint32_t e0 = (kb % NB) * kDK + lane;
 #pragma unroll
             for (int u = 0; u < W; ++u) {
@@ -161,6 +163,36 @@
             }
         }
     };
+    auto qfill = [&](uint32_t g, uint32_t wv, uint32_t nw) {
+        if constexpr (QD) {
+            const uint32_t c0 = (rg * RW + g * kDK) % NP;
+            const uint32_t s0 = (g % kDG) * kDK;
+            const float4* src = m.dtab4 + c0 + lane;
+            if constexpr (SVH_DIAG_QDMA) {
+                for (uint32_t o = wv; o < S; o += nw) {
+                    const uint32_t d = ring_a + (o * kDRS + s0) * 16u;
+                    lds_dma16(src + (size_t)o * NP, d);
+                    if (s0 == 0) lds_dma16(src + (size_t)o * NP, d + kDR * 16u);
+                }
+            } else {
+                constexpr uint32_t kQB = 8;
+                for (uint32_t o0 = wv; o0 < S; o0 += nw * kQB) {
+                    float4 v[kQB];
+#pragma unroll
+                    for (uint32_t r = 0; r < kQB; ++r) v[r] = src[(size_t)min(o0 + r * nw, S - 1) * NP];
+#pragma unroll
+                    for (uint32_t r = 0; r < kQB; ++r) {
+                        const uint32_t o = o0 + r * nw;
+                        if (o < S) {
+                            float* d = ring + ((size_t)o * kDRS + s0 + lane) * 4;
+                            *reinterpret_cast<float4*>(d) = v[r];
+                            if (s0 == 0) *reinterpret_cast<float4*>(d + kDR * 4) = v[r];
+                        }
+                    }
+                }
+            }
+        }
+    };
     if constexpr (LD) {
         if (ldr) {
 #pragma unroll
@@ -179,7 +211,17 @@
     return;
 #endif
     if constexpr (LD) {
-        if (ldr) {
+        if constexpr (QD) {
+            if (ldr) {
+                symloadl(0);
+            } else {
+                qfill(0, w, W);
+                qfill(1, w, W);
+                qfill(2, w, W);
+                qfill(3, w, W);
+            }
+            asm volatile("s_waitcnt vmcnt(0)" ::: "memory");
+        } else if (ldr) {
             gloadl(4);
             symloadl(0);
         } else {
@@ -306,6 +348,14 @@
     };
     auto eread = [&](uint32_t j) {
         const float roff = aq[j % (2 * kAG)];
+        if constexpr (QD) {
+            const f4 e = lds_ld4(__builtin_bit_cast(uint32_t, roff) + lane * 16u);
+            eq[4 * (j % kNE)] = e.x;
+            eq[4 * (j % kNE) + 1] = e.y;
+            eq[4 * (j % kNE) + 2] = e.z;
+            eq[4 * (j % kNE) + 3] = e.w;
+            return;
+        }
         if constexpr (DM == 2) {
             const uint32_t a = __builtin_bit_cast(uint32_t, roff) + lane * 4u;
             eq[4 * (j % kNE)] = lds_ld1(a);
@@ -450,7 +500,7 @@
                     if (SX) gread(xq, xsf, kb, j + kAG);
                 }
                 if (SVH_DIAG_AB == 0 && !FL) {
-                    __builtin_amdgcn_s_waitcnt(0xC07F | (((SX ? 6 : 5) + (PATHS ? 2 : 0) + (DM == 2 ? 2 : 0)) << 8));
+                    __builtin_amdgcn_s_waitcnt(0xC07F | (((SX ? 6 : 5) + (PATHS ? 2 : 0) + (DM == 2 && !QD ? 2 : 0)) << 8));
                     __builtin_amdgcn_sched_barrier(0);
                 }
             }
@@ -497,7 +547,10 @@
         for (uint32_t j = 0; j < rem; ++j) {
             const float4 h = *reinterpret_cast<const float4*>(strm + (e0 + j) * kDE);
             const float roff = adr[e0 + j];
-            if constexpr (DM == 2) {
+            if constexpr (QD) {
+                const f4 e = lds_ld4(__builtin_bit_cast(uint32_t, roff) + lane * 16u);
+                step2(h, SX ? xsf[e0 + j] : 0.0f, (f2){e.x, e.y}, (f2){e.z, e.w});
+            } else if constexpr (DM == 2) {
                 const uint32_t a = __builtin_bit_cast(uint32_t, roff) + lane * 4u;
                 step2(h, SX ? xsf[e0 + j] : 0.0f, (f2){lds_ld1(a), lds_ld1(a + 256u)},
                       (f2){lds_ld1(a + kDRS2 * 4u), lds_ld1(a + kDRS2 * 4u + 256u)});
@@ -511,7 +564,12 @@
     if constexpr (LD) {
         if (ldr) {
             for (uint32_t k = 0; k < nbmax; ++k) {
-                if (!flr) {
+                if constexpr (QD) {
+                    sbuildl(k + 2);
+                    symloadl(k + 3);
+                    qfill(k + 4, 0, 1);
+                    asm volatile("s_waitcnt vmcnt(0)" ::: "memory");
+                } else if (!flr) {
                     sbuildl(k + 2);
                     symloadl(k + 3);
                     lwritel(k + 4);
diff --git a/spec_viterbi_amd/csrc/kernels.h b/spec_viterbi_amd/csrc/kernels.h
--- a/spec_viterbi_amd/csrc/kernels.h
+++ b/spec_viterbi_amd/csrc/kernels.h
@@ -152,12 +152,14 @@
     uint32_t hx_exist;
     uint32_t hl_exist;
     uint32_t ties_heavy;
+    uint32_t dqd;
     unsigned long long* stamps;
     uint32_t diag;
     uint32_t dld;
     const float* dtab2;
     uint32_t nrng2;
     uint32_t dsm;
+    const float4* dtab4;
 };
 constexpr int kPipeStamps = 15;
 constexpr uint32_t kCtrClass = 4, kCtrLeft = 12, kCtrWords = 16;
@@ -201,9 +203,11 @@
 constexpr uint32_t kPQuadStride = 520;
 inline size_t pipe_path_lds_bytes(uint32_t W) { return (size_t)W * 8 * kPQuadStride * 4; }
 uint32_t diag_waves_for(uint64_t nseq);
-size_t diag_lds_bytes(uint32_t W, uint32_t S, uint32_t P, uint32_t dm = 1, bool ld = false);
+size_t diag_lds_bytes(uint32_t W, uint32_t S, uint32_t P, uint32_t dm = 1, bool ld = false, bool quad = false);
 uint32_t diag_sm_for(const PipeModel& m, uint64_t nseq, bool resumed, bool paths);
 bool diag_loader_for(const PipeModel& m, uint64_t nseq, bool resumed, bool paths);
+bool diag_quad_for(const PipeModel& m, uint64_t nseq, bool resumed, bool paths);
+bool diag_quad_table_fits(uint32_t S, uint32_t P, bool sx);
 hipError_t launch_diag(const PipeModel& m, const FusedBatch& b, const PipeScratch& x, hipStream_t stream);
 constexpr uint32_t kDiagSetMaxSym = 32;
 struct DiagSetEntry {
diff --git a/spec_viterbi_amd/csrc/runtime.cpp b/spec_viterbi_amd/csrc/runtime.cpp
--- a/spec_viterbi_amd/csrc/runtime.cpp
+++ b/spec_viterbi_amd/csrc/runtime.cpp
@@ -670,10 +670,24 @@
                 pp.dtab2[((size_t)o * 2) * NP2 + p] = d[0];
                 pp.dtab2[((size_t)o * 2 + 1) * NP2 + p] = d[1];
             }
+        pp.dtab4.resize((size_t)S * NP2 * 4);
+        for (uint32_t o = 0; o < S; ++o) {
+            const float* ea = pp.dtab2.data() + ((size_t)o * 2) * NP2;
+            const float* eb = ea + NP2;
+            float* d = pp.dtab4.data() + (size_t)o * NP2 * 4;
+            for (uint32_t c = 0; c < NP2; ++c) {
+                const uint32_t c2 = (c + 64) % NP2;
+                d[4 * c] = ea[c];
+                d[4 * c + 1] = ea[c2];
+                d[4 * c + 2] = eb[c];
+                d[4 * c + 3] = eb[c2];
+            }
+        }
         if (sh.bw[0] < kInfH) {
             pp.nrng = pp.nrng2 = 0;
             pp.dtab.clear();
             pp.dtab2.clear();
+            pp.dtab4.clear();
         }
     }
     pp.pflags.assign(P, 0);
@@ -776,12 +790,17 @@
             d_dtab2.upload(p.dtab2.data(), p.dtab2.size() * 4, s);
             view.dtab2 = d_dtab2.as<float>();
             view.nrng2 = p.nrng2;
+            if (p.dtab4.size() == (size_t)S * p.P * 4 && diag_quad_table_fits(S, p.P, p.sx)) {
+                d_dtab4.upload(p.dtab4.data(), p.dtab4.size() * 4, s);
+                view.dtab4 = d_dtab4.as<float4>();
+            }
         }
         if (const char* e = std::getenv("SVH_DIAG_SM")) {
             const int v = std::atoi(e);
             view.dsm = v == 1 || v == 2 ? (uint32_t)v : 0u;
         }
         if (const char* e = std::getenv("SVH_DIAG_LOADER"); e && *e) view.dld = std::atoi(e) ? 2u : 1u;
+        if (const char* e = std::getenv("SVH_DIAG_QUAD"); e && *e) view.dqd = std::atoi(e) ? 2u : 1u;
     }
     view.emax2 = p.emax2;
     view.tm = !p.wide && p.SM == 2 && (p.W == 4 || (p.W == 8 && pipe_tm_supported(-8))) && S <= kPairSymbols ? 4u : 0u;
@@ -1357,9 +1376,10 @@
     spec_level = level;
 }
 
-svh_model_info Model::info(uint32_t nseq, bool paths, uint32_t level) const {
+svh_model_info Model::info(uint32_t nseq, bool paths, uint32_t level, uint64_t* quad_lds) const {
     svh_model_info i;
     std::memset(&i, 0, sizeof(i));
+    if (quad_lds) *quad_lds = 0;
     const bool steps = level <= 1 || spec_level < 2;
     const bool pq = paths && steps;
     const PassPlan pl = resolve(nseq, pq, level, nseq != 0 && pq == paths);
@@ -1424,6 +1444,8 @@
         if (!pq) {
             i.diag_sm = (int32_t)diag_sm_for(pipe.view, nseq, false, false);
             i.lds_bytes = diag_lds_bytes(w, host.S, pipe.plan.P, (uint32_t)i.diag_sm, diag_loader_for(pipe.view, nseq, false, false));
+            if (quad_lds && diag_quad_for(pipe.view, nseq, false, false))
+                *quad_lds = diag_lds_bytes(w, host.S, pipe.plan.P, 2, true, true);
         } else {
             i.diag_sm = 1;
             i.lds_bytes = diag_paths_lds_bytes(w, host.S, pipe.plan.sx);
diff --git a/spec_viterbi_amd/csrc/runtime.h b/spec_viterbi_amd/csrc/runtime.h
--- a/spec_viterbi_amd/csrc/runtime.h
+++ b/spec_viterbi_amd/csrc/runtime.h
@@ -129,6 +129,7 @@
     uint32_t nrng = 0;
     std::vector<float> dtab2;
     uint32_t nrng2 = 0;
+    std::vector<float> dtab4;
     float emax2 = 0.0f;
     std::vector<uint8_t> pflags;
     std::vector<int32_t> spos;
@@ -139,7 +140,7 @@
 
 struct DevicePipePlan {
     PipePlan plan;
-    DeviceBuffer d_tab, d_e0, d_start, d_lrow, d_hc, d_stamps, d_pflags, d_spos, d_dtab, d_dtab2;
+    DeviceBuffer d_tab, d_e0, d_start, d_lrow, d_hc, d_stamps, d_pflags, d_spos, d_dtab, d_dtab2, d_dtab4;
     PipeModel view{};
     void upload(const PipePlan& p, uint32_t n, uint32_t S, hipStream_t s);
     void report_stamps(uint32_t nseq) const;
@@ -224,7 +225,7 @@
     const DevicePipePlan& pipe_plan(const PassPlan& p) const { return p.step == StepKernel::PipeWide ? pipe_wide : pipe; }
     const DevicePlan* fused_plan(bool paths) const;
     void spec_build(uint32_t level, hipStream_t s);
-    svh_model_info info(uint32_t nseq = 0, bool paths = false, uint32_t level = 0) const;
+    svh_model_info info(uint32_t nseq = 0, bool paths = false, uint32_t level = 0, uint64_t* quad_lds = nullptr) const;
     void launch_steps(const FusedBatch& b, const PassPlan& p, hipStream_t s) const;
 };
 
diff --git a/spec_viterbi_amd/csrc/svh_api.cpp b/spec_viterbi_amd/csrc/svh_api.cpp
--- a/spec_viterbi_amd/csrc/svh_api.cpp
+++ b/spec_viterbi_amd/csrc/svh_api.cpp
@@ -319,6 +319,14 @@
     return guarded([&] {
         require(b && info, "null argument");
         *info = b->get()->model->info(b->get()->nseq, b->get()->paths, level);
+    });
+}
+
+int svh_batch_diag_quad(svh_batch_t b, uint32_t level, int32_t* quad, uint64_t* lds_bytes) {
+    return guarded([&] {
+        require(b && quad && lds_bytes, "null argument");
+        b->get()->model->info(b->get()->nseq, b->get()->paths, level, lds_bytes);
+        *quad = *lds_bytes ? 1 : 0;
     });
 }
 
diff --git a/spec_viterbi_amd/viterbi.py b/spec_viterbi_amd/viterbi.py
--- a/spec_viterbi_amd/viterbi.py
+++ b/spec_viterbi_amd/viterbi.py
@@ -172,7 +172,12 @@
     def plan(self, level: int = 0) -> dict:
         i = _lib.svh_model_info()
         _lib.check(_lib.lib.svh_batch_plan(self._h, int(level), ctypes.byref(i)))
-        return {name: getattr(i, name) for name, _ in i._fields_}
+        plan = {name: getattr(i, name) for name, _ in i._fields_}
+        quad, lds = ctypes.c_int32(), ctypes.c_uint64()
+        _lib.check(_lib.lib.svh_batch_diag_quad(self._h, int(level), ctypes.byref(quad), ctypes.byref(lds)))
+        plan["diag_quad"] = int(quad.value)
+        plan["diag_quad_lds_bytes"] = int(lds.value)
+        return plan
 
     def fallbacks(self) -> int:
         r = ctypes.c_uint64()
```

Result: faster. 3.675 million M state-updates/s (median of 6 runs) (+13.2%).
